# quickwit-oss/tantivy

Hardware: AMD Instinct MI355X
Metric: queries_per_sec_2term_AND_bm25_top10 (higher is better)
Workload: dtype u32+f32; 1 GPU; and2: 10000 queries/batch, k=10, one 10M-doc Zipf segment per GPU (256 terms, df_r=0.5N/r, WithFreqs); term ranks ~ Zipf(1); distinct_queries=3877, mode=block-max pruned (block_wand_intersection semantics), exchange=single rank: no exchange, segments_per_gpu=1, index_bytes=40381332

## Files before the change

tantivy_amd/csrc/tq_api.cpp:

```cpp
#include "tq_internal.hpp"
#include "../host/bm25.hpp"

namespace tqi {

thread_local std::string g_last_error;

int fail(int code, const char *fmt, ...) {
  char buf[512];
  va_list ap;
  va_start(ap, fmt);
  vsnprintf(buf, sizeof buf, fmt, ap);
  va_end(ap);
  g_last_error = buf;
  return code;
}
}

int tq_internal_fail(int code, const char *where, const char *what) {
  return fail(code, "%s: %s", where, what);
}
bool tq_internal_ctx_has_device(const tq_ctx *ctx, int device) {
  return std::find(ctx->devices.begin(), ctx->devices.end(), device) != ctx->devices.end();
}

extern "C" {

const char *tq_last_error(void) { return g_last_error.c_str(); }

int tq_init(const int *device_ids, int n_devices, tq_ctx **out) {
  if (!out) return fail(TQ_ERR_INVALID, "tq_init: out is null");
  int count = 0;
  hipError_t e = hipGetDeviceCount(&count);
  if (e != hipSuccess || count == 0)
    return fail(TQ_ERR_NO_DEVICE, "tq_init: no HIP device visible (%s)",
                e == hipSuccess ? "count=0" : hipGetErrorString(e));
  tq_ctx *ctx = new tq_ctx();
  if (!device_ids || n_devices <= 0) {
    ctx->devices.push_back(0);
  } else {
    for (int i = 0; i < n_devices; ++i) {
      if (device_ids[i] < 0 || device_ids[i] >= count) {
        delete ctx;
        return fail(TQ_ERR_INVALID, "tq_init: device %d out of range (%d visible)", device_ids[i],
                    count);
      }
      ctx->devices.push_back(device_ids[i]);
    }
  }
  *out = ctx;
  return TQ_OK;
}

void tq_shutdown(tq_ctx *ctx) { delete ctx; }

static int segment_upload_common(tq_ctx *ctx, int device, uint32_t max_doc, const uint8_t *idx,
                                 size_t idx_len, const uint8_t *pos, size_t pos_len,
                                 const uint8_t *fieldnorm, size_t fn_len, uint8_t record_option,
                                 bool from_device, tq_segment **out) {
  if (!ctx || !out || !idx) return fail(TQ_ERR_INVALID, "tq_segment_upload: null argument");
  if (idx_len < 8) return fail(TQ_ERR_FORMAT, "idx sub-file shorter than its 8-byte header");
  if (record_option > TQ_WITH_FREQS_AND_POSITIONS)
    return fail(TQ_ERR_INVALID, "bad record_option %u", record_option);
  if (fieldnorm && fn_len < max_doc)
    return fail(TQ_ERR_FORMAT, "fieldnorm file has %zu bytes for max_doc %u", fn_len, max_doc);
  if (std::find(ctx->devices.begin(), ctx->devices.end(), device) == ctx->devices.end())
    return fail(TQ_ERR_INVALID, "device %d not part of this context", device);
  HIP_TRY(hipSetDevice(device));
  tq_segment *s = new tq_segment();
  s->submit = tq_new_submit_queue();
  if (!s->submit) {
    delete s;
    return fail(TQ_ERR_INVALID, "tq_segment_upload: out of memory");
  }
  s->ctx = ctx;
  s->device = device;
  s->dscratch = ctx->scratch_for(device);
  s->max_doc = max_doc;
  s->record_option = record_option;
  s->idx_len = idx_len;
  s->pos_len = (pos && pos_len) ? pos_len : 0;
  if (!from_device) {
    s->h_idx.assign(idx, idx + idx_len);
    if (pos && pos_len) s->h_pos.assign(pos, pos + pos_len);
  }
  const hipMemcpyKind kind = from_device ? hipMemcpyDeviceToDevice : hipMemcpyHostToDevice;
  auto up = [&](uint8_t **dst, const uint8_t *src, size_t n) -> int {
    HIP_TRY(hipMalloc((void **)dst, n + PAD));
    HIP_TRY(hipMemset(*dst + n, 0, PAD));
    HIP_TRY(hipMemcpy(*dst, src, n, kind));
    return TQ_OK;
  };
  int rc = up(&s->d_idx, idx, idx_len);
  if (rc == TQ_OK && pos && pos_len) rc = up(&s->d_pos, pos, pos_len);
  if (rc == TQ_OK && fieldnorm) rc = up(&s->d_fn, fieldnorm, max_doc);
  if (rc == TQ_OK) {
    hipError_t e = hipStreamCreateWithFlags(&s->stream, hipStreamNonBlocking);
    if (e == hipSuccess) e = hipEventCreateWithFlags(&s->ev_stage_done, hipEventDisableTiming);
    if (e == hipSuccess) e = hipEventCreateWithFlags(&s->ev_fork, hipEventDisableTiming);
    if (e == hipSuccess) e = hipEventCreateWithFlags(&s->ev_join, hipEventDisableTiming);
    if (e == hipSuccess) e = hipEventCreateWithFlags(&s->ev_batch_done, hipEventDisableTiming);
    if (e == hipSuccess) e = hipStreamCreateWithFlags(&s->side_stream, hipStreamNonBlocking);
    if (e == hipSuccess) e = hipStreamCreateWithFlags(&s->copy_stream, hipStreamNonBlocking);
    for (int i = 0; i < 2 && e == hipSuccess; ++i) {
      e = hipEventCreateWithFlags(&s->ev_copy_done[i], hipEventDisableTiming);
      if (e == hipSuccess) e = hipEventCreateWithFlags(&s->ev_buf_free[i], hipEventDisableTiming);
    }
    for (int i = 0; i < tq_segment::kTimingRing; ++i) {
      if (e == hipSuccess) e = hipEventCreate(&s->ev_t0[i]);
      if (e == hipSuccess) e = hipEventCreate(&s->ev_t1[i]);
      if (e == hipSuccess) e = hipEventCreate(&s->ev_k0[i]);
      if (e == hipSuccess) e = hipEventCreate(&s->ev_k1[i]);
    }
    if (e == hipSuccess) e = hipMalloc((void **)&s->d_match_counter, 6u * sizeof(unsigned long long));
    if (e == hipSuccess) e = hipMalloc((void **)&s->d_tp_info, 2 * sizeof(TqpInfo));
    if (e != hipSuccess) rc = fail(TQ_ERR_HIP, "segment setup: %s", hipGetErrorString(e));
  }
  if (rc != TQ_OK) {
    tq_segment_free(s);
    return rc;
  }
  s->dseg.idx = s->d_idx;
  s->dseg.pos = s->d_pos;
  s->dseg.fieldnorm = s->d_fn;
  s->dseg.max_doc = max_doc;
  s->dseg.const_fieldnorm_id = 1;
  s->dseg.min_fieldnorm_id = 1;
  if (fieldnorm && !from_device) {
    uint8_t mn = 255;
    for (uint32_t d = 0; d < max_doc; ++d) mn = fieldnorm[d] < mn ? fieldnorm[d] : mn;
    s->dseg.min_fieldnorm_id = max_doc ? mn : 0;
  } else if (fieldnorm) {
    uint32_t *slot = (uint32_t *)s->d_tp_info;
    uint32_t mn = 255;
    hipError_t e = hipMemcpy(slot, &mn, 4, hipMemcpyHostToDevice);
    if (e == hipSuccess) e = tqp_launch_min_fieldnorm(s->d_fn, max_doc, slot, s->stream);
    if (e == hipSuccess) e = hipMemcpyAsync(&mn, slot, 4, hipMemcpyDeviceToHost, s->stream);
    if (e == hipSuccess) e = hipStreamSynchronize(s->stream);
    if (e != hipSuccess) {
      tq_segment_free(s);
      return fail(TQ_ERR_HIP, "fieldnorm scan: %s", hipGetErrorString(e));
    }
    s->dseg.min_fieldnorm_id = max_doc ? mn : 0;
  }
  {
    uint64_t total_tokens = 0;
    hipError_t e = hipSuccess;
    if (!from_device)
      memcpy(&total_tokens, idx, 8);
    else
      e = hipMemcpy(&total_tokens, s->d_idx, 8, hipMemcpyDeviceToHost);
    const float avg = max_doc ? (float)total_tokens / (float)max_doc : 0.0f;
    if (e == hipSuccess && total_tokens && std::isfinite(avg) && avg > 0.0f) {
      const tantivy_amd::Bm25Weight w = tantivy_amd::Bm25Weight::from_idf(1.0f, avg);
      e = hipMalloc((void **)&s->d_local_cache, 256 * sizeof(float));
      if (e == hipSuccess) e = hipMemcpy(s->d_local_cache, w.cache, 256 * sizeof(float), hipMemcpyHostToDevice);
    }
    if (e != hipSuccess) {
      tq_segment_free(s);
      return fail(TQ_ERR_HIP, "segment cache: %s", hipGetErrorString(e));
    }
  }
  *out = s;
  return TQ_OK;
}

int tq_segment_upload(tq_ctx *ctx, int device, uint32_t max_doc, const uint8_t *idx,
                      size_t idx_len, const uint8_t *pos, size_t pos_len, const uint8_t *fieldnorm,
                      size_t fn_len, uint8_t record_option, tq_segment **out) {
  return segment_upload_common(ctx, device, max_doc, idx, idx_len, pos, pos_len, fieldnorm, fn_len,
                               record_option, false, out);
}

int tq_segment_upload_device(tq_ctx *ctx, int device, uint32_t max_doc, const uint8_t *d_idx,
                             size_t idx_len, const uint8_t *d_pos, size_t pos_len,
                             const uint8_t *d_fieldnorm, size_t fn_len, uint8_t record_option,
                             tq_segment **out) {
  return segment_upload_common(ctx, device, max_doc, d_idx, idx_len, d_pos, pos_len, d_fieldnorm,
                               fn_len, record_option, true, out);
}

int tq_segment_upload_fields(tq_ctx *ctx, int device, uint32_t max_doc, uint32_t n_fields, const tq_field_files *fields,
                             uint8_t record_option, tq_segment **out) {
  if (!ctx || !out || !fields) return fail(TQ_ERR_INVALID, "tq_segment_upload_fields: null argument");
  if (n_fields == 0 || n_fields > TQ_MAX_FIELDS)
    return fail(TQ_ERR_INVALID, "tq_segment_upload_fields: n_fields %u not in 1..%u", n_fields, TQ_MAX_FIELDS);
  if (n_fields == 1)
    return tq_segment_upload(ctx, device, max_doc, fields[0].idx, fields[0].idx_len, fields[0].pos, fields[0].pos_len,
                             fields[0].fieldnorm, fields[0].fn_len, record_option, out);
  uint64_t idx_base[TQ_MAX_FIELDS], pos_base[TQ_MAX_FIELDS], pos_len[TQ_MAX_FIELDS];
  size_t idx_total = 0, pos_total = 0;
  for (uint32_t f = 0; f < n_fields; ++f) {
    const tq_field_files &ff = fields[f];
    if (!ff.idx) return fail(TQ_ERR_INVALID, "tq_segment_upload_fields: field %u: null idx", f);
    if (ff.idx_len < 8) return fail(TQ_ERR_FORMAT, "field %u: idx sub-file shorter than its 8-byte header", f);
    if (ff.fieldnorm && ff.fn_len < max_doc)
      return fail(TQ_ERR_FORMAT, "field %u: fieldnorm file has %zu bytes for max_doc %u", f, ff.fn_len, max_doc);
    pos_len[f] = ff.pos && ff.pos_len ? ff.pos_len : 0;
    idx_base[f] = idx_total;
    pos_base[f] = pos_total;
    idx_total += f + 1 < n_fields ? (ff.idx_len + PAD + 15) & ~(size_t)15 : ff.idx_len;
    pos_total += f + 1 < n_fields && pos_len[f] ? (pos_len[f] + PAD + 15) & ~(size_t)15 : pos_len[f];
  }
  std::vector<uint8_t> idx(idx_total, 0), pos(pos_total, 0);
  for (uint32_t f = 0; f < n_fields; ++f) {
    memcpy(idx.data() + idx_base[f], fields[f].idx, fields[f].idx_len);
    if (pos_len[f]) memcpy(pos.data() + pos_base[f], fields[f].pos, pos_len[f]);
  }
  tq_segment *s = nullptr;
  int rc = segment_upload_common(ctx, device, max_doc, idx.data(), idx_total, pos_total ? pos.data() : nullptr, pos_total,
                                 fields[0].fieldnorm, fields[0].fn_len, record_option, false, &s);
  if (rc != TQ_OK) return rc;
  s->n_fields = n_fields;
  for (uint32_t f = 0; f < n_fields; ++f) {
    s->field_idx_base[f] = idx_base[f];
    s->field_idx_len[f] = fields[f].idx_len;
    s->field_pos_base[f] = pos_base[f];
    s->field_pos_len[f] = pos_len[f];
    if (f == 0 || !fields[f].fieldnorm) continue;
    hipError_t e = hipMalloc((void **)&s->d_fn_field[f], (size_t)max_doc + PAD);
    if (e == hipSuccess) e = hipMemset(s->d_fn_field[f] + max_doc, 0, PAD);
    if (e == hipSuccess) e = hipMemcpy(s->d_fn_field[f], fields[f].fieldnorm, max_doc, hipMemcpyHostToDevice);
    if (e != hipSuccess) {
      tq_segment_free(s);
      return fail(TQ_ERR_HIP, "field %u fieldnorms: %s", f, hipGetErrorString(e));
    }
  }
  *out = s;
  return TQ_OK;
}

void tq_segment_free(tq_segment *s) {
  if (!s) return;
  (void)hipSetDevice(s->device);
  if (s->stream) (void)hipStreamSynchronize(s->stream);
  if (s->batch_in_flight && s->ev_batch_done) (void)hipEventSynchronize(s->ev_batch_done);
  for (void *slab : s->term_slabs) (void)hipFree(slab);
  dense_arena_free(s);
  for (void *ptr : s->dense_extra) (void)hipFree(ptr);
  if (s->d_terms) (void)hipFree(s->d_terms);
  if (s->d_idx) (void)hipFree(s->d_idx);
  if (s->d_pos) (void)hipFree(s->d_pos);
  if (s->d_fn) (void)hipFree(s->d_fn);
  for (uint8_t *fn : s->d_fn_field)
    if (fn) (void)hipFree(fn);
  if (s->d_alive) (void)hipFree(s->d_alive);
  if (s->d_docmat) (void)hipFree(s->d_docmat);
  if (s->d_doccls) (void)hipFree(s->d_doccls);
  if (s->d_tp_info) (void)hipFree(s->d_tp_info);
  if (s->d_local_cache) (void)hipFree(s->d_local_cache);
  if (s->d_match_counter) (void)hipFree(s->d_match_counter);
  s->d_stage.release();
  s->d_misc.release();
  for (int i = 0; i < 2; ++i) {
    s->h_prep_stage[i].release();
    if (s->ev_prep[i]) (void)hipEventDestroy(s->ev_prep[i]);
  }
  if (s->ev_prep_order) (void)hipEventDestroy(s->ev_prep_order);
  s->d_thr.release();
  tq_free_plan_scratch(s->plan);
  s->plan = nullptr;
  tq_free_submit_queue(s->submit);
  s->submit = nullptr;
  s->d_qmatches.release();
  s->d_share_words.release();
  s->d_ashare_words.release();
  s->d_bshare_words.release();
  s->d_count_queries.release();
  s->d_count_out.release();
  s->d_count_bits.release();
  s->d_count_wgs.release();
  s->d_set_work.release();
  free_columns(s);
  s->d_docset_queries.release();
  s->d_docset_counts.release();
  s->d_docset_offs.release();
  s->d_docset_partials.release();
  s->d_docset_starts.release();
  s->d_docset_docs.release();
  s->d_docset_squeries.release();
  s->d_docset_caches.release();
  s->d_docset_scores.release();
  s->d_docset_trees.release();
  s->d_sort_ks.release();
  s->d_sort_partials.release();
  s->d_sort_slice_counts.release();
  s->d_sort_rows.release();
  s->h_sort_ks.release();
  s->d_agg_rows.release();
  s->d_agg_term_rows.release();
  s->d_agg_range_starts.release();
  s->h_agg_range_starts.release();
  s->h_docset.release();
  s->h_stage.release();
  s->h_out.release();
  if (s->side_stream) (void)hipStreamSynchronize(s->side_stream);
  if (s->copy_stream) (void)hipStreamSynchronize(s->copy_stream);
  for (hipEvent_t ev : {s->ev_stage_done, s->ev_fork, s->ev_join, s->ev_batch_done, s->ev_copy_done[0],
                        s->ev_copy_done[1], s->ev_buf_free[0], s->ev_buf_free[1]})
    if (ev) (void)hipEventDestroy(ev);
  if (s->side_stream) (void)hipStreamDestroy(s->side_stream);
  if (s->copy_stream) (void)hipStreamDestroy(s->copy_stream);
  s->d_stage_alt.release();
  for (int i = 0; i < tq_segment::kTimingRing; ++i)
    for (hipEvent_t ev : {s->ev_t0[i], s->ev_t1[i], s->ev_k0[i], s->ev_k1[i]})
      if (ev) (void)hipEventDestroy(ev);
  if (s->stream) (void)hipStreamDestroy(s->stream);
  delete s;
}

}

namespace tqi {
int order_after_last_batch(tq_segment *s, hipStream_t st) {
  if (s->batch_in_flight && s->last_stream != st)
    HIP_TRY(hipStreamWaitEvent(st, s->ev_batch_done, 0));
  return TQ_OK;
}
int wait_segment_idle(tq_segment *s) {
  HIP_TRY(hipStreamSynchronize(s->stream));
  if (s->batch_in_flight) {
    HIP_TRY(hipEventSynchronize(s->ev_batch_done));
    s->batch_in_flight = false;
  }
  return TQ_OK;
}
}

extern "C" {

int tq_segment_set_alive_bitset(tq_segment *s, const uint8_t *bytes, size_t len) {
  if (!s) return fail(TQ_ERR_INVALID, "tq_segment_set_alive_bitset: null segment");
  TQ_SEGMENT_LOCK(s);
  HIP_TRY(hipSetDevice(s->device));
  {
    const int wrc = wait_segment_idle(s);
    if (wrc != TQ_OK) return wrc;
  }
  if (s->d_alive) (void)hipFree(s->d_alive);
  s->d_alive = nullptr;
  s->bytes_alive = 0;
  s->dseg.alive = nullptr;
  if (!bytes) return TQ_OK;
  if (len < 4) return fail(TQ_ERR_FORMAT, "alive bitset shorter than its header");
  const uint32_t max_value = rd32(bytes);
  const size_t need = ((size_t)s->max_doc + 63) / 64 * 8;
  if (max_value != s->max_doc || len - 4 < need || (len - 4) % 8 != 0)
    return fail(TQ_ERR_FORMAT, "alive bitset for %u docs / %zu bytes does not fit max_doc %u",
                max_value, len - 4, s->max_doc);
  HIP_TRY(hipMalloc((void **)&s->d_alive, len - 4 + PAD));
  HIP_TRY(hipMemset(s->d_alive + (len - 4), 0, PAD));
  HIP_TRY(hipMemcpy(s->d_alive, bytes + 4, len - 4, hipMemcpyHostToDevice));
  s->bytes_alive = len - 4;
  s->dseg.alive = s->d_alive;
  s->alive_docs = 0;
  for (uint32_t d = 0; d + 8u <= s->max_doc; d += 8u) s->alive_docs += (uint32_t)__builtin_popcount(bytes[4 + (d >> 3)]);
  if (s->max_doc & 7u) s->alive_docs += (uint32_t)__builtin_popcount(bytes[4 + (s->max_doc >> 3)] & ((1u << (s->max_doc & 7u)) - 1u));
  return TQ_OK;
}

int tq_last_batch_match_counts(tq_segment *s, uint32_t *out, uint32_t n) {
  if (!s || !out) return fail(TQ_ERR_INVALID, "tq_last_batch_match_counts: null argument");
  TQ_SEGMENT_LOCK(s);
  if (n > s->last_batch_queries) return fail(TQ_ERR_INVALID, "the last batch had %u queries", s->last_batch_queries);
  HIP_TRY(hipSetDevice(s->device));
  {
    const int wrc = wait_segment_idle(s);
    if (wrc != TQ_OK) return wrc;
  }
  HIP_TRY(hipMemcpy(out, s->d_qmatches.p, (size_t)n * sizeof(uint32_t), hipMemcpyDeviceToHost));
  return TQ_OK;
}

int tq_last_batch_query_kernels(tq_segment *s, uint32_t *out, uint32_t n) {
  if (!s || !out) return fail(TQ_ERR_INVALID, "tq_last_batch_query_kernels: null argument");
  TQ_SEGMENT_LOCK(s);
  if (!s->opt.record_query_kernels || s->last_query_kernel.size() < n)
    return fail(TQ_ERR_INVALID, "the last batch recorded %zu queries (option \"record_query_kernels\")", s->last_query_kernel.size());
  memcpy(out, s->last_query_kernel.data(), (size_t)n * sizeof(uint32_t));
  return TQ_OK;
}

int tq_count_batch(tq_segment *s, const tq_query *queries, uint32_t n_queries,
                   uint32_t *out_counts) {
  if (!s || (!queries && n_queries) || !out_counts)
    return fail(TQ_ERR_INVALID, "tq_count_batch: null argument");
  TQ_SEGMENT_LOCK(s);
  if (n_queries == 0) return TQ_OK;
  return count_batch(s, queries, n_queries, out_counts);
}

static DocsetCall rows_call(const char *fn, uint32_t *out_docs, float *out_scores, uint64_t out_cap, uint64_t *out_starts) {
  DocsetCall call(fn);
  call.out_docs = out_docs;
  call.out_scores = out_scores;
  call.out_cap = out_cap;
  call.out_starts = out_starts;
  return call;
}

int tq_docset_batch(tq_segment *s, const tq_query *queries, uint32_t n_queries, uint32_t *out_docs, uint64_t out_cap,
                    uint64_t *out_starts) {
  if (!s || (!queries && n_queries) || (!out_docs && out_cap) || !out_starts)
    return fail(TQ_ERR_INVALID, "tq_docset_batch: null argument");
  TQ_SEGMENT_LOCK(s);
  return docset_batch(s, queries, n_queries, rows_call("tq_docset_batch", out_docs, nullptr, out_cap, out_starts));
}

int tq_docset_batch_device(tq_segment *s, const tq_query *queries, uint32_t n_queries, uint32_t *d_out_docs,
                           uint64_t out_cap, uint64_t *d_out_starts, void *hip_stream) {
  if (!s || (!queries && n_queries) || (!d_out_docs && out_cap) || !d_out_starts)
    return fail(TQ_ERR_INVALID, "tq_docset_batch_device: null argument");
  TQ_SEGMENT_LOCK(s);
  DocsetCall call = rows_call("tq_docset_batch_device", d_out_docs, nullptr, out_cap, d_out_starts);
  call.device_out = true;
  call.hip_stream = hip_stream;
  return docset_batch(s, queries, n_queries, call);
}

int tq_docset_scored_batch(tq_segment *s, const tq_query *queries, uint32_t n_queries, uint32_t *out_docs, float *out_scores,
                           uint64_t out_cap, uint64_t *out_starts) {
  if (!s || (!queries && n_queries) || ((!out_docs || !out_scores) && out_cap) || !out_starts)
    return fail(TQ_ERR_INVALID, "tq_docset_scored_batch: null argument");
  TQ_SEGMENT_LOCK(s);
  DocsetCall call = rows_call("tq_docset_scored_batch", out_docs, out_scores, out_cap, out_starts);
  call.scored = true;
  return docset_batch(s, queries, n_queries, call);
}

int tq_docset_scored_batch_device(tq_segment *s, const tq_query *queries, uint32_t n_queries, uint32_t *d_out_docs,
                                  float *d_out_scores, uint64_t out_cap, uint64_t *d_out_starts, void *hip_stream) {
  if (!s || (!queries && n_queries) || ((!d_out_docs || !d_out_scores) && out_cap) || !d_out_starts)
    return fail(TQ_ERR_INVALID, "tq_docset_scored_batch_device: null argument");
  TQ_SEGMENT_LOCK(s);
  DocsetCall call = rows_call("tq_docset_scored_batch_device", d_out_docs, d_out_scores, out_cap, d_out_starts);
  call.scored = call.device_out = true;
  call.hip_stream = hip_stream;
  return docset_batch(s, queries, n_queries, call);
}

int tq_last_batch_stats(tq_segment *s, tq_batch_stats *out) {
  if (!s || !out) return fail(TQ_ERR_INVALID, "tq_last_batch_stats: null argument");
  TQ_SEGMENT_LOCK(s);
  HIP_TRY(hipSetDevice(s->device));
  if (s->stats_pending) {
    {
      const int wrc = wait_segment_idle(s);
      if (wrc != TQ_OK) return wrc;
    }
    unsigned long long m = 0;
    if (s->stats_sorted) {
      unsigned long long t[3] = {0, 0, 0};
      HIP_TRY(hipMemcpy(t, s->d_match_counter, sizeof t, hipMemcpyDeviceToHost));
      m = t[0];
      s->stats.matches = m;
      s->stats.algorithmic_bytes += 8u * t[1] + (s->stats_sorted_optional ? 8u * t[0] : 0u) + 13u * t[2];
      if (s->stats_agg_metric) {
        unsigned long long b[2] = {0, 0};
        HIP_TRY(hipMemcpy(b, s->d_match_counter + 3, sizeof b, hipMemcpyDeviceToHost));
        s->stats.algorithmic_bytes += 8u * b[0] + (s->stats_agg_metric_optional ? 8u * b[1] : 0u);
      }
      if (s->stats_agg_terms) {
        unsigned long long e = 0;
        HIP_TRY(hipMemcpy(&e, s->d_match_counter + 3, sizeof e, hipMemcpyDeviceToHost));
        s->stats.algorithmic_bytes += 12u * e;
        if (s->stats_agg_terms_sub) {
          unsigned long long b[2] = {0, 0};
          HIP_TRY(hipMemcpy(b, s->d_match_counter + 4, sizeof b, hipMemcpyDeviceToHost));
          s->stats.algorithmic_bytes += 40u * e + 8u * b[0] + (s->stats_agg_metric_optional ? 8u * b[1] : 0u);
        }
        if (s->stats_agg_terms_hist_row) {
          unsigned long long b[2] = {0, 0};
          HIP_TRY(hipMemcpy(b, s->d_match_counter + 4, sizeof b, hipMemcpyDeviceToHost));
          s->stats.algorithmic_bytes += 4u * (uint64_t)(s->stats_agg_terms_hist_row - 1u) * e + 8u * b[0] + (s->stats_agg_metric_optional ? 8u * b[1] : 0u);
        }
      }
      s->stats_sorted = false;
    } else {
      HIP_TRY(hipMemcpy(&m, s->d_match_counter, sizeof m, hipMemcpyDeviceToHost));
      s->stats.matches = m;
      s->stats.algorithmic_bytes += m * s->stats_match_bytes;
    }
    if (s->opt.timing) {
      uint64_t first = s->batches_reported;
      if (s->batches_timed - first > (uint64_t)tq_segment::kTimingRing)
        first = s->batches_timed - tq_segment::kTimingRing;
      double k_sum = 0, t_sum = 0;
      uint32_t n = 0;
      for (uint64_t b = first; b < s->batches_timed; ++b) {
        const int i = (int)(b % tq_segment::kTimingRing);
        float km = 0, tm = 0;
        if (hipEventElapsedTime(&km, s->ev_k0[i], s->ev_k1[i]) == hipSuccess &&
            hipEventElapsedTime(&tm, s->ev_t0[i], s->ev_t1[i]) == hipSuccess) {
          k_sum += km;
          t_sum += tm;
          ++n;
        }
      }
      s->batches_reported = s->batches_timed;
      if (n) {
        s->stats.kernel_ms = (float)(k_sum / n);
        s->stats.total_ms = (float)(t_sum / n);
      }
      s->stats.batches_averaged = n;
    }
    s->stats.host_plan_ms = s->host_ms_n ? (float)(s->host_ms_sum / s->host_ms_n) : 0.0f;
    s->host_ms_sum = 0;
    s->host_ms_n = 0;
    s->stats_pending = false;
  }
  *out = s->stats;
  return TQ_OK;
}

int tq_segment_reserve_columns(tq_segment *s, const uint64_t *postings_offs, uint32_t n) {
  if (!s || (!postings_offs && n)) return fail(TQ_ERR_INVALID, "tq_segment_reserve_columns: null argument");
  TQ_SEGMENT_LOCK(s);
  if (!s->terms.empty())
    return fail(TQ_ERR_INVALID, "tq_segment_reserve_columns: call it before the first tq_term_prepare");
  s->reserved_cols.clear();
  for (uint32_t i = 0; i < n && i < TQD_MAT_SLOTS; ++i) s->reserved_cols[postings_offs[i]] = true;
  s->cols_reserved = true;
  return TQ_OK;
}

int tq_segment_get_stats(tq_segment *s, tq_segment_stats *out) {
  if (!s || !out) return fail(TQ_ERR_INVALID, "tq_segment_get_stats: null argument");
  TQ_SEGMENT_LOCK(s);
  tq_segment_stats r{};
  r.index_bytes = s->idx_len;
  r.positions_bytes = s->pos_len;
  r.fieldnorm_bytes = s->d_fn ? s->max_doc : 0;
  r.alive_bytes = s->bytes_alive;
  r.term_table_bytes = s->bytes_term_tables + s->d_terms_cap * sizeof(TqdTerm);
  r.bitmap_bytes = s->bytes_bitmaps;
  r.docmat_bytes = s->bytes_docmat;
  r.posdir_bytes = s->bytes_posdir;
  r.scratch_bytes = s->d_stage.cap + s->d_stage_alt.cap + s->d_misc.cap + s->d_thr.cap + s->d_qmatches.cap + s->d_share_words.cap +
                    s->d_ashare_words.cap + s->d_bshare_words.cap + s->d_count_queries.cap + s->d_count_out.cap +
                    s->d_count_bits.cap + s->d_count_wgs.cap + s->d_set_work.cap + s->docset_scratch_bytes();
  {
    std::lock_guard<std::mutex> lk(s->dscratch->m);
    r.device_scratch_bytes = s->dscratch->partials.cap + s->dscratch->share_stage.cap + s->dscratch->ashare_stage.cap +
                             s->dscratch->bshare_stage.cap;
  }
  r.n_terms = (uint32_t)s->terms.size();
  r.n_dense_lists = s->n_dense_lists;
  r.n_docmat_columns = s->n_mat_slots;
  r.probe_evictions = (uint32_t)std::min<uint64_t>(s->probe_evictions, 0xFFFFFFFFull);
  r.dense_budget_bytes = s->dense_budget();
  r.lead_mat_bytes = s->lmat_bytes_total;
  r.lead_mat_stale = s->lmat_stale_skips;
  *out = r;
  return TQ_OK;
}

int tq_set_option(tq_segment *s, const char *name, int64_t value) {
  if (!s || !name) return fail(TQ_ERR_INVALID, "tq_set_option: null argument");
  TQ_SEGMENT_LOCK(s);
  if (!strcmp(name, "exhaustive"))
    __atomic_store_n(&s->opt.exhaustive, value != 0 ? 1 : 0, __ATOMIC_RELAXED);
  else if (!strcmp(name, "timing"))
    s->opt.timing = value != 0;
  else if (!strcmp(name, "use_dpp"))
    s->opt.use_dpp = value != 0;
  else if (!strcmp(name, "use_dense"))
    s->opt.use_dense = value != 0;
  else if (!strcmp(name, "or_windows"))
    s->opt.or_windows = value < 0 ? -1 : (value != 0);
  else if (!strcmp(name, "dense_ratio") && value >= 1)
    s->opt.dense_ratio = (int)value;
  else if (!strcmp(name, "rdir_budget_x") && value >= 0 && value <= 0x7FFFFFFF)
    s->opt.rdir_budget_x = (int)value;
  else if (!strcmp(name, "lead_mat_budget_x") && value >= 0 && value <= 0x7FFFFFFF)
    s->opt.lead_mat_budget_x = (int)value;
  else if (!strcmp(name, "lead_mat_cut") && value >= 1 && value <= 0x7FFFFFFF)
    s->opt.lead_mat_cut = (int)value;
  else if (!strcmp(name, "probe_budget_x") && value >= 0 && value <= 0x7FFFFFFF)
    s->opt.probe_budget_x = (int)value, s->probe_full = false;
  else if (!strcmp(name, "dense_budget_x") && value >= 0)
    s->opt.dense_budget_x = (int)value;
  else if (!strcmp(name, "bound_slack_ppm") && value >= 0 && value <= 1000000000)
    __atomic_store_n(&s->opt.bound_slack_ppm, (int)value, __ATOMIC_RELAXED);
  else if (!strcmp(name, "dense"))
    s->opt.dense = value != 0;
  else if (!strcmp(name, "docmat"))
    s->opt.docmat = value != 0;
  else if (!strcmp(name, "docsig"))
    s->opt.docsig = value != 0;
  else if (!strcmp(name, "device_prepare"))
    s->opt.device_prepare = value != 0;
  else if (!strcmp(name, "xunion_ratio") && value >= 0 && value <= 0x7FFFFFFF)
    s->opt.xunion_ratio = (int)value;
  else if (!strcmp(name, "count_bitmap_ratio") && value >= 0 && value <= 0x7FFFFFFF)
    s->opt.count_bitmap_ratio = (int)value;
  else if (!strcmp(name, "docset_temp_lists") && value >= 0 && value <= 0x7FFFFFFF)
    s->opt.docset_temp_lists = (int)value;
  else if (!strcmp(name, "docset_trees") && (value == 0 || value == 1))
    s->opt.docset_trees = (int)value;
  else if (!strcmp(name, "docset_score_trees") && (value == 0 || value == 1))
    s->opt.docset_score_trees = (int)value;
  else if (!strcmp(name, "sort_slices") && value >= 0 && value <= 256)
    s->opt.sort_slices = (int)value;
  else if (!strcmp(name, "agg_slices") && value >= 0 && value <= 256)
    s->opt.agg_slices = (int)value;
  else if (!strcmp(name, "agg_lds_buckets") && value >= 0 && value <= (int64_t)tqk_agg_lds_buckets())
    s->opt.agg_lds_buckets = (int)value;
  else if (!strcmp(name, "ashare_inline_warm") && value >= 0 && value <= 2)
    s->opt.ashare_inline_warm = (int)value;
  else if (!strcmp(name, "ashare_min_batch") && value >= 0 && value <= 0x7FFFFFFF)
    s->opt.ashare_min_batch = (int)value;
  else if (!strcmp(name, "xunion_min_queries") && value >= 1 && value <= 0x7FFFFFFF)
    s->opt.xunion_min_queries = (int)value;
  else if (!strcmp(name, "record_query_kernels"))
    s->opt.record_query_kernels = value != 0;
  else if (!strcmp(name, "debug") && value >= -1 && value <= 0x7FFFFFFF)
    s->opt.debug = (int)value;
  else if (!strcmp(name, "submit_window_us") && value >= 0 && value <= 1000000)
    s->opt.submit_window_us = (int)value;
  else
    return fail(TQ_ERR_INVALID, "unknown option '%s'", name);
  return TQ_OK;
}

int tq_decode_postings(tq_segment *s, tq_term_handle term, uint32_t *docs, uint32_t *tfs) {
  if (!s || !docs || !tfs) return fail(TQ_ERR_INVALID, "tq_decode_postings: null argument");
  TQ_SEGMENT_LOCK(s);
  if (term >= s->terms.size()) return fail(TQ_ERR_INVALID, "unknown term handle %u", term);
  if (s->terms[term].set_kind != TermHost::kNoSet) return fail(TQ_ERR_INVALID, "tq_decode_postings: handle %u is a term set: it has no postings", term);
  HIP_TRY(hipSetDevice(s->device));
  int rc = sync_terms(s, s->stream);
  if (rc != TQ_OK) return rc;
  const TermHost &t = s->terms[term];
  const size_t bytes = (size_t)t.doc_freq * sizeof(uint32_t);
  rc = s->d_misc.ensure(2 * bytes + 64);
  if (rc != TQ_OK) return rc;
  uint32_t *dd = (uint32_t *)s->d_misc.p, *dt = dd + t.doc_freq;
  hipError_t e = tqk_launch_decode_list(s->dseg, s->d_terms, term, t.n_blocks, dd, dt,
                                        s->opt.use_dpp != 0, s->stream);
  if (e != hipSuccess) return fail(TQ_ERR_HIP, "decode launch: %s", hipGetErrorString(e));
  HIP_TRY(hipMemcpyAsync(docs, dd, bytes, hipMemcpyDeviceToHost, s->stream));
  HIP_TRY(hipMemcpyAsync(tfs, dt, bytes, hipMemcpyDeviceToHost, s->stream));
  HIP_TRY(hipStreamSynchronize(s->stream));
  return TQ_OK;
}

int tq_decode_position_deltas(tq_segment *s, tq_term_handle term, uint32_t *out, uint64_t cap,
                              uint64_t *n_out) {
  if (!s || !n_out) return fail(TQ_ERR_INVALID, "tq_decode_position_deltas: null argument");
  TQ_SEGMENT_LOCK(s);
  if (term >= s->terms.size()) return fail(TQ_ERR_INVALID, "unknown term handle %u", term);
  const TermHost &t = s->terms[term];
  if (t.set_kind != TermHost::kNoSet) return fail(TQ_ERR_INVALID, "tq_decode_position_deltas: handle %u is a term set: it has no positions", term);
  if (t.positions_len == 0) return fail(TQ_ERR_UNSUPPORTED, "term has no positions on the device");
  *n_out = t.n_positions;
  const uint64_t n = std::min<uint64_t>(cap, t.n_positions);
  if (n == 0 || !out) return TQ_OK;
  HIP_TRY(hipSetDevice(s->device));
  int rc = sync_terms(s, s->stream);
  if (rc != TQ_OK) return rc;
  rc = s->d_misc.ensure(n * sizeof(uint32_t));
  if (rc != TQ_OK) return rc;
  hipError_t e = tqk_launch_decode_positions(s->dseg, s->d_terms, term, (uint32_t *)s->d_misc.p, n,
                                             s->stream);
  if (e != hipSuccess) return fail(TQ_ERR_HIP, "decode launch: %s", hipGetErrorString(e));
  HIP_TRY(hipMemcpyAsync(out, s->d_misc.p, n * sizeof(uint32_t), hipMemcpyDeviceToHost, s->stream));
  HIP_TRY(hipStreamSynchronize(s->stream));
  return TQ_OK;
}

namespace {
struct TableSpan {
  const void *p = nullptr;
  size_t bytes = 0;
  bool host = false;
};
bool table_span(tq_segment *s, uint32_t term, uint32_t which, TableSpan &sp) {
  if (which >= TQ_TABLE_DOCMAT) {
    const size_t per_doc = (size_t)s->max_doc * sizeof(uint64_t);
    switch (which) {
      case TQ_TABLE_DOCMAT: sp = {s->d_docmat, s->d_docmat ? per_doc : 0, false}; return true;
      case TQ_TABLE_DOCCLS: sp = {s->d_doccls, s->d_doccls ? per_doc : 0, false}; return true;
      case TQ_TABLE_LOCAL_CACHE: sp = {s->d_local_cache, s->d_local_cache ? 256 * sizeof(float) : 0, false}; return true;
      case TQ_TABLE_MIN_FIELDNORM_ID: sp = {&s->dseg.min_fieldnorm_id, sizeof(uint32_t), true}; return true;
      default: return false;
    }
  }
  const TermHost &t = s->terms[term];
  const TqdTerm &d = s->h_dterms[term];
  const size_t n_words = bitmap_words(s);
  const size_t n_dir = ((size_t)t.doc_freq + 3) / 4 + 1;
// ... 185 lines not shown
```

tantivy_amd/csrc/tq_count.cpp:

```cpp
#include "tq_internal.hpp"

#include <deque>
#include <unordered_map>

namespace tqi {

int parse_flat_clauses(tq_segment *s, const tq_query &q, FlatClauses &fc, const char **why) {
  fc.n_cl = fc.n_must = fc.n_should = 0;
  fc.empty = fc.all_based = fc.all_boost_mixed = false;
  fc.msm = 0;
  *why = "";
  if (query_has_all(q)) {
    AllForm f;
    const int arc = all_query_form(q, f, why);
    if (arc != TQ_OK) return arc == TQ_ERR_UNSUPPORTED ? FLAT_UNSUPPORTED : FLAT_INVALID;
    AllView v;
    all_strip_view(q, f, v);
    const int prc = parse_flat_clauses(s, v.q, fc, why);
    if (prc != FLAT_OK) return prc;
    for (uint32_t c = 0; c < fc.n_cl; ++c)
      for (uint32_t i = 0; i < fc.cl[c].n; ++i) fc.cl[c].pos[i] = v.pos[fc.cl[c].pos[i]];
    fc.all_based = f.kind == TQ_ALL_BASED;
    fc.all_base = f.base;
    fc.all_boost_mixed = f.boost_mixed;
    return FLAT_OK;
  }
  fc.msm = q.mode == TQ_MODE_BOOL ? q.min_should_match : 0u;
  if (!q.terms || q.n_terms == 0 || q.n_terms > TQ_MAX_TERMS) return *why = "n_terms out of range (1..TQ_MAX_TERMS) or no terms", FLAT_INVALID;
  if (q.mode == TQ_MODE_PHRASE) return *why = "a phrase query", FLAT_UNSUPPORTED;
  if (q.mode > TQ_MODE_BOOL) return *why = "unknown mode", FLAT_INVALID;
  if (q.mode == TQ_MODE_BOOL && !q.occurs) return *why = "TQ_MODE_BOOL without occurs", FLAT_INVALID;
  if (bool_query_is_tree(q)) return *why = "a nested boolean query", FLAT_UNSUPPORTED;
  FlatClauses::Clause *cl = fc.cl;
  uint32_t n_cl = 0;
  for (uint32_t i = 0; i < q.n_terms; ++i) {
    uint32_t occur = q.mode == TQ_MODE_AND ? TQ_MUST : TQ_SHOULD;
    uint32_t id = i;
    if (q.mode == TQ_MODE_BOOL) {
      occur = q.occurs[i];
      if (occur > TQ_MUST_NOT) return *why = "occur out of range", FLAT_INVALID;
      if (q.clause_of) id = q.clause_of[i];
    }
    uint32_t c = 0;
    while (c < n_cl && cl[c].id != id) ++c;
    if (c == n_cl) {
      cl[n_cl] = FlatClauses::Clause{};
      cl[n_cl].id = id;
      cl[n_cl].occur = occur;
      ++n_cl;
    } else if (cl[c].occur != occur) {
      return *why = "mixed occurs in one clause", FLAT_INVALID;
    }
    const uint32_t h = q.terms[i];
    if (h == TQ_TERM_ABSENT) continue;
    if (h >= s->terms.size()) return *why = "term handle out of range", FLAT_INVALID;
    cl[c].pos[cl[c].n] = i;
    cl[c].terms[cl[c].n++] = h;
    cl[c].cost += s->terms[h].doc_freq;
  }
  fc.n_cl = n_cl;
  for (uint32_t c = 0; c < n_cl; ++c) {
    if (cl[c].occur == TQ_MUST) {
      if (cl[c].n == 0) fc.empty = true;
      ++fc.n_must;
    } else if (cl[c].n) {
      if (cl[c].occur == TQ_SHOULD) ++fc.n_should;
    }
  }
  return FLAT_OK;
}

bool count_expression(tq_segment *s, const tq_query &q, TqkCountQuery &cq, bool &known, uint64_t &driver_postings,
                      std::unordered_map<uint32_t, uint32_t> &temp_slot, uint32_t max_temp) {
  known = false;
  driver_postings = 0;
  cq = TqkCountQuery{};
  FlatClauses fc;
  const char *why;
  if (parse_flat_clauses(s, q, fc, &why) != FLAT_OK) return false;
  using Clause = FlatClauses::Clause;
  const Clause *cl = fc.cl;
  const uint32_t n_cl = fc.n_cl, n_must = fc.n_must, n_should = fc.n_should;
  bool empty = fc.empty;
  for (uint32_t c = 0; c < n_cl; ++c)
    for (uint32_t i = 0; i < cl[c].n; ++i) {
      const uint32_t h = cl[c].terms[i];
      if (!expression_bitmap(s, s->terms[h]) && !temp_slot.count(h) && temp_slot.size() >= max_temp) return false;
    }
  if (fc.all_based) return false;
  uint32_t msm = fc.msm;
  if (msm > n_should) empty = true;
  bool should_is_must = false;
  if (!empty && msm >= 2) {
    if (msm != n_should) return false;
    should_is_must = true;
    msm = 0;
  }
  if (n_must == 0 && n_should == 0) empty = true;
  if (empty) {
    known = true;
    return true;
  }
  uint32_t n = 0;
  uint64_t must_cost = ~0ull, should_cost = 0;
  auto put = [&](const Clause &c, uint32_t kind, bool clause_union) {
    for (uint32_t i = 0; i < c.n; ++i) {
      const TermHost &th = s->terms[c.terms[i]];
      if (expression_bitmap(s, th)) {
        cq.dense[n] = (const uint2 *)th.dense_blob;
      } else {
        const uint32_t slot = temp_slot.emplace(c.terms[i], (uint32_t)temp_slot.size()).first->second;
        cq.dense[n] = (const uint2 *)(uintptr_t)slot;
        cq.narrow |= 1u << n;
      }
      cq.kinds |= kind << (2u * n);
      if (kind == TQK_COUNT_MUST && (!clause_union || i + 1 == c.n)) cq.clause_end |= 1u << n;
      ++n;
    }
  };
  const bool has_must = n_must > 0 || should_is_must;
  for (uint32_t c = 0; c < n_cl; ++c) {
    if (cl[c].occur == TQ_MUST || (should_is_must && cl[c].occur == TQ_SHOULD && cl[c].n)) {
      put(cl[c], TQK_COUNT_MUST, true);
      must_cost = std::min(must_cost, cl[c].cost);
    }
  }
  for (uint32_t c = 0; c < n_cl; ++c)
    if (cl[c].occur == TQ_MUST_NOT && cl[c].n) put(cl[c], TQK_COUNT_NOT, false);
  if (!should_is_must)
    for (uint32_t c = 0; c < n_cl; ++c)
      if (cl[c].occur == TQ_SHOULD && cl[c].n) {
        if (has_must && msm == 0) continue;
        put(cl[c], TQK_COUNT_SHOULD, false);
        should_cost += cl[c].cost;
      }
  cq.n_terms = n;
  cq.flags = (has_must ? TQK_COUNT_HAS_MUST : 0u) | ((has_must && msm == 1) ? TQK_COUNT_NEED_SHOULD : 0u);
  driver_postings = has_must ? must_cost : should_cost;
  return true;
}

int count_batch(tq_segment *s, const tq_query *queries, uint32_t n_queries, uint32_t *out_counts) {
  static const uint32_t kRatioEnv = tune_u32("TQ_COUNT_BITMAP_RATIO", 0xFFFFFFFFu);
  const uint32_t kRatio = kRatioEnv != 0xFFFFFFFFu ? kRatioEnv : (uint32_t)s->opt.count_bitmap_ratio;
  static const uint64_t kTempBudget = (uint64_t)std::max<uint32_t>(1u, tune_u32("TQ_COUNT_TEMP_MB", 1024)) << 20;
  const uint32_t n_words = (uint32_t)(((uint64_t)s->max_doc + 31u) / 32u);
  const uint32_t words_per_list = (n_words + 63u) & ~63u;
  const uint32_t max_temp = (uint32_t)std::min<uint64_t>(4096u, kTempBudget / ((uint64_t)words_per_list * 4u));
  std::vector<TqkCountQuery> cqs;
  std::vector<uint32_t> bitmap_q, scan_q, all_q;
  std::unordered_map<uint32_t, uint32_t> temp_slot, trial;
  std::deque<AllView> views;
  std::vector<tq_query> eff;
  std::vector<uint8_t> done;
  const tq_query *const given = queries;
  s->last_batch_slop = false;
  for (uint32_t qi = 0; qi < n_queries; ++qi) {
    if (!query_has_all(given[qi])) continue;
    if (eff.empty()) {
      eff.assign(given, given + n_queries);
      done.assign(n_queries, 0);
    }
    AllForm f;
    const char *why = "";
    const int arc = all_query_form(given[qi], f, &why);
    if (arc != TQ_OK) return fail(arc, "tq_count_batch: query %u: %s", qi, why);
    views.emplace_back();
    all_strip_view(given[qi], f, views.back());
    eff[qi] = views.back().q;
    if (f.kind != TQ_ALL_BASED) continue;
    done[qi] = 1;
    bool any_not = false;
    for (uint32_t i = 0; i < given[qi].n_terms; ++i) {
      if (!((f.keep_mask >> i) & 1u)) continue;
      if (given[qi].terms[i] >= s->terms.size()) return fail(TQ_ERR_INVALID, "tq_count_batch: query %u: term handle out of range", qi);
      any_not = any_not || (given[qi].occurs && given[qi].occurs[i] == TQ_MUST_NOT);
    }
    if (f.min_should == 0 && !any_not)
      out_counts[qi] = s->d_alive ? s->alive_docs : s->max_doc;
    else
      all_q.push_back(qi);
  }
  if (!eff.empty()) queries = eff.data();
  for (uint32_t qi = 0; qi < n_queries; ++qi) {
    if (!given[qi].slop) continue;
    SlopView sv;
    const int vrc = slop_view(s, given[qi], qi, "tq_count_batch", sv, false);
    if (vrc != TQ_OK) return vrc;
    if (done.empty()) done.assign(n_queries, 0);
    done[qi] = 1;
    all_q.push_back(qi);
  }
  std::vector<uint8_t> set_q;
  for (uint32_t qi = 0; s->n_set_slots && qi < n_queries; ++qi) {
    bool has = false;
    const int src = check_set_query(s, given[qi], qi, "tq_count_batch", &has);
    if (src != TQ_OK) return src;
    if (has && set_q.empty()) set_q.assign(n_queries, 0);
    if (has) set_q[qi] = 1;
  }
  for (uint32_t qi = 0; s->n_field_terms && qi < n_queries; ++qi)
    if (query_names_field(s, given[qi])) {
      const int frc = check_field_query(s, given[qi], qi, "tq_count_batch");
      if (frc != TQ_OK) return frc;
    }
  for (uint32_t qi = 0; qi < n_queries; ++qi) {
    if (!done.empty() && done[qi]) continue;
    TqkCountQuery cq;
    bool known = false;
    uint64_t driver = 0;
    trial = temp_slot;
    const bool names_set = !set_q.empty() && set_q[qi];
    const bool expr = (kRatio || names_set) && count_expression(s, queries[qi], cq, known, driver, trial, max_temp);
    if (expr && known) {
      out_counts[qi] = 0;
    } else if (expr && (names_set || driver * kRatio >= (uint64_t)cq.n_terms * s->max_doc)) {
      cqs.push_back(cq);
      bitmap_q.push_back(qi);
      temp_slot.swap(trial);
    } else if (names_set) {
      TqkDocsetQuery dq;
      const char *why = "";
      const int drc = docset_expression(s, given[qi], dq, &why);
      if (drc != FLAT_OK) return fail(drc == FLAT_UNSUPPORTED ? TQ_ERR_UNSUPPORTED : TQ_ERR_INVALID, "tq_count_batch: query %u: %s", qi, why);
      all_q.push_back(qi);
    } else {
      scan_q.push_back(qi);
    }
  }
  HIP_TRY(hipSetDevice(s->device));
  uint32_t mask = 0;
  uint64_t algo_bytes = 0;
  if (!scan_q.empty()) {
    const uint32_t n = (uint32_t)scan_q.size();
    std::vector<tq_query> qs(n);
    for (uint32_t i = 0; i < n; ++i) {
      qs[i] = queries[scan_q[i]];
      qs[i].k = 1;
    }
    std::vector<float> sc(n);
    std::vector<uint32_t> dc(n), ct(n), mc(n);
    CallOpts co;
    int rc = resolve_opts(s, nullptr, co);
    if (rc != TQ_OK) return rc;
    co.exhaustive = true;
    rc = search_batch_host(s, qs.data(), n, 1, sc.data(), dc.data(), ct.data(), co);
    if (rc != TQ_OK) return rc;
    rc = tq_last_batch_match_counts(s, mc.data(), n);
    if (rc != TQ_OK) return rc;
    for (uint32_t i = 0; i < n; ++i) out_counts[scan_q[i]] = mc[i];
    mask = s->stats.kernel_mask;
    algo_bytes = s->stats.algorithmic_bytes;
  } else {
    const int wrc = wait_segment_idle(s);
    if (wrc != TQ_OK) return wrc;
  }
  if (!bitmap_q.empty()) {
    const uint32_t n = (uint32_t)bitmap_q.size();
    int rc = s->d_count_queries.ensure((size_t)n * sizeof(TqkCountQuery));
    if (rc == TQ_OK) rc = s->d_count_out.ensure((size_t)n * sizeof(uint32_t));
    if (rc != TQ_OK) return rc;
    if (!temp_slot.empty()) {
      const int src = sync_terms(s, s->stream);
      if (src != TQ_OK) return src;
      std::vector<uint4> wgs;
      for (const auto &kv : temp_slot) push_scatter_work(wgs, s, kv.first, kv.second);
      rc = s->d_count_bits.ensure((size_t)temp_slot.size() * words_per_list * sizeof(uint32_t));
      if (rc == TQ_OK) rc = s->d_count_wgs.ensure(wgs.size() * sizeof(uint4));
      if (rc != TQ_OK) return rc;
      HIP_TRY(hipMemsetAsync(s->d_count_bits.p, 0, (size_t)temp_slot.size() * words_per_list * sizeof(uint32_t), s->stream));
      HIP_TRY(hipMemcpyAsync(s->d_count_wgs.p, wgs.data(), wgs.size() * sizeof(uint4), hipMemcpyHostToDevice, s->stream));
      const hipError_t se = tqk_launch_count_scatter(s->dseg, s->d_terms, (const uint4 *)s->d_count_wgs.p, (uint32_t)wgs.size(),
                                                     (uint32_t *)s->d_count_bits.p, words_per_list, s->stream);
      if (se != hipSuccess) return fail(TQ_ERR_HIP, "count scatter launch: %s", hipGetErrorString(se));
      for (TqkCountQuery &cq : cqs)
        for (uint32_t m = 0; m < cq.n_terms; ++m)
          if ((cq.narrow >> m) & 1u)
            cq.dense[m] = (const uint2 *)((const uint32_t *)s->d_count_bits.p + (size_t)(uintptr_t)cq.dense[m] * words_per_list);
    }
    HIP_TRY(hipMemcpyAsync(s->d_count_queries.p, cqs.data(), (size_t)n * sizeof(TqkCountQuery), hipMemcpyHostToDevice, s->stream));
    HIP_TRY(hipMemsetAsync(s->d_count_out.p, 0, (size_t)n * sizeof(uint32_t), s->stream));
    TqkCountParams p{};
    p.queries = (const TqkCountQuery *)s->d_count_queries.p;
    p.alive = s->d_alive;
    p.out_counts = (uint32_t *)s->d_count_out.p;
    p.n_queries = n;
    p.n_words = n_words;
    const hipError_t e = tqk_launch_count_bitmaps(p, s->stream);
    if (e != hipSuccess) return fail(TQ_ERR_HIP, "count kernel launch: %s", hipGetErrorString(e));
    std::vector<uint32_t> got(n);
    HIP_TRY(hipMemcpyAsync(got.data(), s->d_count_out.p, (size_t)n * sizeof(uint32_t), hipMemcpyDeviceToHost, s->stream));
    HIP_TRY(hipStreamSynchronize(s->stream));
    for (uint32_t i = 0; i < n; ++i) {
      out_counts[bitmap_q[i]] = got[i];
      algo_bytes += (uint64_t)cqs[i].n_terms * p.n_words * 4u;
    }
    mask |= TQ_KERNEL_COUNT_BITMAPS;
  }
  if (!all_q.empty()) {
    const uint32_t n = (uint32_t)all_q.size();
    std::vector<tq_query> qs(n);
    for (uint32_t i = 0; i < n; ++i) qs[i] = given[all_q[i]];
    std::vector<uint64_t> starts((size_t)n + 1u);
    DocsetCall call("tq_count_batch", DocsetConsumer::kCount);
    call.out_starts = starts.data();
    call.caller_q = all_q.data();
    call.n_caller = n_queries;
    const int rc = docset_batch(s, qs.data(), n, call);
// ... 15 lines not shown
```

tantivy_amd/csrc/tq_docset.cpp:

```cpp
#include "tq_internal.hpp"

#include <deque>
#include <unordered_map>

namespace tqi {

int docset_expression(tq_segment *s, const tq_query &q, TqkDocsetQuery &dq, const char **why, FlatClauses *fc_out) {
  dq = TqkDocsetQuery{};
  FlatClauses fc_own;
  FlatClauses &fc = fc_out ? *fc_out : fc_own;
  const int prc = parse_flat_clauses(s, q, fc, why);
  if (prc != FLAT_OK) return prc;
  using Clause = FlatClauses::Clause;
  if (fc.empty_set()) {
    dq.min_should = 1;
    return FLAT_OK;
  }
  const bool should_is_must = fc.should_is_must();
  const uint32_t msm = should_is_must ? 0u : fc.msm;
  const bool has_must = fc.n_must > 0 || should_is_must || fc.all_based;
  uint32_t n = 0;
  auto put = [&](const Clause &c, uint32_t kind) {
    for (uint32_t i = 0; i < c.n; ++i) {
      const TermHost &th = s->terms[c.terms[i]];
// ... 374 lines not shown
    if (b.tree_bytes) memcpy(h_tq, b.tqs.data(), b.tree_bytes);
    if (tree_map_bytes) {
      uint32_t *const map = (uint32_t *)(h_tq + b.tree_bytes);
      for (const DocsetSubBatch &sb : b.cut.subs)
        for (uint32_t t = sb.t0; t < sb.t1; ++t) map[t] = b.tree_q[t] - sb.q0;
    }
    if (slop_bytes) memcpy(h_tq + b.slop_off, b.slop_qs.data(), slop_bytes);
    HIP_TRY(hipMemcpyAsync(s->d_docset_trees.p, h_tq, tree_blob_bytes, hipMemcpyHostToDevice, st));
  }
  if (call.consumer == Consumer::kSort) rc = sort_prepare(s, *call.sort, b.queries, n_queries, b.cut.max_sub_n, b.n_words, st);
  if (call.consumer == Consumer::kAgg) rc = agg_prepare(s, *call.agg, n_queries, b.cut.max_sub_n, b.n_words, st);
  if (rc != TQ_OK) return rc;
  if (slop_bytes) {
    HIP_TRY(hipMemsetAsync(s->d_slop_over.p, 0, (size_t)b.n_over_words() * sizeof(uint32_t), st));
    s->last_batch_slop = true;
  }
  return TQ_OK;
}

int launch_match_bits(const Batch &b, const DocsetSubBatch &sb) {
  tq_segment *const s = b.s;
  if (sb.wg1 > sb.wg0) {
    HIP_TRY(hipMemsetAsync(s->d_count_bits.p, 0, (size_t)sb.n_temp * b.words_per_list * sizeof(uint32_t), b.st));
    const int rc = launched(tqk_launch_count_scatter(s->dseg, s->d_terms, (const uint4 *)s->d_count_wgs.p + sb.wg0, (uint32_t)(sb.wg1 - sb.wg0),
                                                     (uint32_t *)s->d_count_bits.p, b.words_per_list, b.st), "doc-set scatter");
    if (rc != TQ_OK) return rc;
  }
  if (sb.t1 > sb.t0) {
    TqkDocsetTreeParams tp{};
    tp.seg = s->dseg;
    tp.terms = s->d_terms;
    tp.queries = (const TqdTreeQuery *)s->d_docset_trees.p + sb.t0;
    tp.table_base = (const uint8_t *)s->share_table_lo;
    tp.bits = (uint32_t *)s->d_count_bits.p;
    tp.n_queries = sb.t1 - sb.t0;
    tp.n_words = b.n_words;
    tp.words_per_list = b.words_per_list;
    tp.any_phrase = sb.any_phrase ? 1u : 0u;
    const int rc = launched(tqk_launch_docset_tree(tp, b.st), "doc-set tree");
    if (rc != TQ_OK) return rc;
  }
  if (sb.s1 > sb.s0) {
    TqkPhraseSlopParams pp{};
    pp.seg = s->dseg;
    pp.terms = s->d_terms;
    pp.queries = (const TqdSlopQuery *)((const uint8_t *)s->d_docset_trees.p + b.slop_off) + sb.s0;
    pp.table_base = (const uint8_t *)s->share_table_lo;
    pp.overflow = (uint32_t *)s->d_slop_over.p;
    pp.bits = (uint32_t *)s->d_count_bits.p;
    pp.n_queries = sb.s1 - sb.s0;
    pp.n_words = b.n_words;
    pp.words_per_list = b.words_per_list;
    for (uint32_t k = sb.s0; k < sb.s1; ++k) (b.slop_qs[k].n_terms > 2u ? pp.any_carry : pp.any_pair) = 1u;
    return launched(tqk_launch_phrase_slop_bits(pp, b.st), "sloppy phrase");
  }
  return TQ_OK;
}

hipError_t launch_scores(const Batch &b, const DocsetSubBatch &sb, const TqkDocsetParams &p, float *d_scores) {
  tq_segment *const s = b.s;
  TqkScoreParams sp{};
  sp.seg = s->dseg;
  sp.terms = s->d_terms;
  sp.caches = (const float *)s->d_docset_caches.p;
  sp.out_docs = p.out_docs;
  sp.out_scores = d_scores;
  sp.out_cap = p.out_cap;
  sp.n_tiles = b.n_tiles;
  sp.any_blocks = sb.score_blocks ? 1u : 0u;
  hipError_t e = hipSuccess;
  uint32_t r0 = sb.q0;
  for (uint32_t t = sb.t0; t <= sb.t1 && e == hipSuccess; ++t) {
    const uint32_t r1 = t < sb.t1 ? b.tree_q[t] : sb.q1;
    if (r1 > r0) {
      sp.queries = (const TqkScoreQuery *)s->d_docset_squeries.p + r0;
      sp.tile_counts = p.tile_counts + (size_t)(r0 - sb.q0) * b.n_tiles;
      sp.tile_offs = p.tile_offs + (size_t)(r0 - sb.q0) * b.n_tiles;
      sp.n_queries = r1 - r0;
      if (b.score_fields) {
        TqkScoreFieldsParams fp{};
        fp.base = sp;
        fp.fn[0] = s->d_fn;
        for (uint32_t f = 1; f < TQK_MAX_FIELDS; ++f) fp.fn[f] = s->d_fn_field[f];
        e = tqk_launch_docset_score_fields(fp, b.st);
      } else {
        e = tqk_launch_docset_score(sp, b.st);
      }
    }
    r0 = r1 + 1u;
  }
  if (e != hipSuccess || sb.t1 == sb.t0) return e;
  TqkDocsetTreeScoreParams tsp{};
  tsp.seg = s->dseg;
  tsp.terms = s->d_terms;
  tsp.queries = (const TqdTreeQuery *)s->d_docset_trees.p + sb.t0;
  tsp.query_of = (const uint32_t *)((const uint8_t *)s->d_docset_trees.p + b.tree_bytes) + sb.t0;
  tsp.caches = sp.caches;
  tsp.table_base = (const uint8_t *)s->share_table_lo;
  tsp.tile_counts = p.tile_counts;
  tsp.tile_offs = p.tile_offs;
  tsp.out_docs = p.out_docs;
  tsp.out_scores = d_scores;
  tsp.out_cap = p.out_cap;
  tsp.n_queries = sb.t1 - sb.t0;
  tsp.n_tiles = b.n_tiles;
  tsp.any_phrase = sb.any_phrase ? 1u : 0u;
  return tqk_launch_docset_tree_score(tsp, b.st);
}

int launch_consumer(const Batch &b, const DocsetSubBatch &sb, uint32_t stages, uint32_t *d_docs, float *d_scores, uint64_t cap) {
  static const uint32_t kStageMin = tune_u32("TQ_DOCSET_STAGE_MIN", 2048);
  tq_segment *const s = b.s;
  TqkDocsetParams p{};
  p.queries = (const TqkDocsetQuery *)s->d_docset_queries.p + sb.q0;
  p.alive = s->d_alive;
  p.tile_counts = (uint32_t *)s->d_docset_counts.p;
  p.tile_offs = (uint64_t *)s->d_docset_offs.p;
  p.partials = (uint64_t *)s->d_docset_partials.p;
  p.base_in = sb.q0 ? b.d_starts + sb.q0 : nullptr;
  p.out_starts = b.d_starts + sb.q0;
  p.query_sizes = (uint32_t *)s->d_qmatches.p + sb.q0;
  p.total_out = s->d_match_counter;
  p.out_docs = d_docs;
  p.out_cap = cap;
  p.n_queries = sb.q1 - sb.q0;
  p.n_tiles = b.n_tiles;
  p.n_words = b.n_words;
  p.max_doc = s->max_doc;
  p.stage_min_docs = kStageMin;
  if (b.call.consumer == Consumer::kSort) return sort_launch(s, *b.call.sort, p, sb.q0, b.st);
  if (b.call.consumer == Consumer::kAgg) return agg_launch(s, *b.call.agg, p, sb.q0, b.st);
  hipError_t e = hipSuccess;
  if (stages & DS_COUNT) {
    e = tqk_launch_docset_count(p, b.st);
    if (e == hipSuccess) e = tqk_launch_docset_scan(p, b.st);
  }
  if (e == hipSuccess && (stages & DS_WRITE)) e = tqk_launch_docset_write(p, b.st);
  if (e == hipSuccess && (stages & DS_WRITE) && b.call.scored) e = launch_scores(b, sb, p, d_scores);
  return launched(e, "doc-set kernel");
}

int sweep(const Batch &b, uint32_t stages, uint32_t *d_docs, float *d_scores, uint64_t cap) {
  for (const DocsetSubBatch &sb : b.cut.subs) {
    int rc = (stages & DS_SCATTER) ? launch_match_bits(b, sb) : TQ_OK;
    if (rc == TQ_OK) rc = launch_consumer(b, sb, stages, d_docs, d_scores, cap);
    if (rc != TQ_OK) return rc;
  }
  return TQ_OK;
}

int run_device(const Batch &b) {
  tq_segment *const s = b.s;
  const DocsetCall &call = b.call;
  if (b.timed) HIP_TRY(hipEventRecord(s->ev_k0[b.ring], b.st));
  int rc = sweep(b, DS_SCATTER | DS_COUNT | DS_WRITE, call.out_docs, call.out_scores, call.out_cap);
  if (rc == TQ_OK && call.consumer == Consumer::kAgg) rc = agg_finish(s, *call.agg, b.n_queries, b.st);
  if (rc != TQ_OK) return rc;
  if (b.timed) {
    HIP_TRY(hipEventRecord(s->ev_k1[b.ring], b.st));
    HIP_TRY(hipEventRecord(s->ev_t1[b.ring], b.st));
    ++s->batches_timed;
  }
  s->stats_pending = true;
  s->stats_match_bytes = call.scored ? 9 : 4;
  s->stats_sorted = !b.own_passes();
  s->stats_sorted_optional = (call.sort && call.sort->optional) || (call.agg && call.agg->optional);
  s->stats_agg_metric = call.agg && call.agg->metric;
  s->stats_agg_metric_optional = call.agg && call.agg->metric_optional;
  s->stats_agg_terms = call.agg && call.agg->terms;
  s->stats_agg_terms_sub = call.agg && call.agg->terms_sub;
  s->stats_agg_terms_hist_row = call.agg && call.agg->terms_hist ? call.agg->plan.n_buckets + 1u : 0u;
  HIP_TRY(hipEventRecord(s->ev_batch_done, b.st));
  s->last_stream = b.st;
  s->batch_in_flight = true;
  return TQ_OK;
}

int run_host(const Batch &b) {
  tq_segment *const s = b.s;
  const DocsetCall &call = b.call;
  const std::vector<DocsetSubBatch> &subs = b.cut.subs;
  int rc = sweep(b, DS_SCATTER | DS_COUNT, nullptr, nullptr, 0);
  if (rc != TQ_OK) return rc;
  HIP_TRY(hipMemcpyAsync(call.out_starts, b.d_starts, ((size_t)b.n_queries + 1u) * sizeof(uint64_t), hipMemcpyDeviceToHost, b.st));
  HIP_TRY(hipStreamSynchronize(b.st));
  const uint64_t total = call.out_starts[b.n_queries];
  s->stats.matches = total;
  if (call.consumer == Consumer::kCount) return slop_overflow_readback(s, call.fn);
  s->stats.algorithmic_bytes += (call.scored ? 9u : 4u) * total;
  if (total > call.out_cap)
    return fail(TQ_ERR_INVALID, "%s: the batch has %llu docs, out_cap is %llu (out_starts is filled: retry with that many)", call.fn,
                (unsigned long long)total, (unsigned long long)call.out_cap);
  if (!total) return slop_overflow_readback(s, call.fn);
  rc = s->d_docset_docs.ensure((size_t)total * sizeof(uint32_t));
  if (rc == TQ_OK && call.scored) rc = s->d_docset_scores.ensure((size_t)total * sizeof(float));
  if (rc != TQ_OK) return rc;
  if (subs.size() > 1 && !b.slop_qs.empty())
    HIP_TRY(hipMemsetAsync(s->d_slop_over.p, 0, (size_t)b.n_over_words() * sizeof(uint32_t), b.st));
  rc = sweep(b, subs.size() == 1 ? DS_WRITE : (DS_SCATTER | DS_COUNT | DS_WRITE), (uint32_t *)s->d_docset_docs.p, (float *)s->d_docset_scores.p, total);
  if (rc != TQ_OK) return rc;
  HIP_TRY(hipMemcpyAsync(call.out_docs, s->d_docset_docs.p, (size_t)total * sizeof(uint32_t), hipMemcpyDeviceToHost, b.st));
  if (call.scored) HIP_TRY(hipMemcpyAsync(call.out_scores, s->d_docset_scores.p, (size_t)total * sizeof(float), hipMemcpyDeviceToHost, b.st));
  HIP_TRY(hipStreamSynchronize(b.st));
  if (s->d_docset_docs.cap > ((size_t)256 << 20)) s->d_docset_docs.release();
  if (s->d_docset_scores.cap > ((size_t)256 << 20)) s->d_docset_scores.release();
  return slop_overflow_readback(s, call.fn);
}

}

int docset_batch(tq_segment *s, const tq_query *queries, uint32_t n_queries, const DocsetCall &call) {
  static const uint64_t kTempBudget = (uint64_t)std::max<uint32_t>(1u, tune_u32("TQ_COUNT_TEMP_MB", 1024)) << 20;
  Batch b{s, queries, n_queries, call};
  b.n_words = (uint32_t)(((uint64_t)s->max_doc + 31u) / 32u);
  b.words_per_list = (b.n_words + 63u) & ~63u;
  b.n_tiles = (b.n_words + tqk_docset_tile_words() - 1u) / tqk_docset_tile_words();
  b.max_temp = s->opt.docset_temp_lists > 0
                   ? (uint32_t)s->opt.docset_temp_lists
                   : (uint32_t)std::min<uint64_t>(4096u, kTempBudget / std::max<uint64_t>(1u, (uint64_t)b.words_per_list * 4u));
  b.max_temp = std::max<uint32_t>(b.max_temp, TQ_MAX_TERMS);
  b.max_sub_queries = std::max<uint32_t>(1u, (1u << 26) / std::max(1u, b.n_tiles));
  b.dqs.resize(n_queries);
  b.sqs.resize(call.scored ? n_queries : 0u);
  s->last_batch_slop = false;
  s->slop_over_words = b.n_over_words();
  int rc = check_and_express(b);
  if (rc == TQ_OK) rc = plan_trees(b);
  if (rc != TQ_OK) return rc;
  cut_docset_subs(s, b.dqs, b.sqs, b.tree_q, b.tqs, b.slop_qi, b.slop_qs, b.max_temp, b.max_sub_queries, b.cut);

  HIP_TRY(hipSetDevice(s->device));
  b.st = call.device_out && call.hip_stream ? (hipStream_t)call.hip_stream : s->stream;
  rc = wait_segment_idle(s);
  if (rc != TQ_OK) return rc;
  const bool scored = call.scored;
  s->stats = tq_batch_stats{};
  s->stats.kernel_mask = (call.consumer == Consumer::kSort ? TQ_KERNEL_SORT : call.consumer == Consumer::kAgg ? (call.agg->terms_hist ? TQ_KERNEL_AGG_TERMS_HIST : call.agg->terms_sub ? TQ_KERNEL_AGG_TERMS_SUB : call.agg->terms ? TQ_KERNEL_AGG_TERMS : call.agg->range ? TQ_KERNEL_AGG_RANGE : call.agg->metric ? TQ_KERNEL_AGG_SUB : TQ_KERNEL_AGG) : TQ_KERNEL_DOCSET) |
                         (scored ? TQ_KERNEL_DOCSET_SCORE : 0u) | (b.tqs.empty() ? 0u : TQ_KERNEL_DOCSET_TREE) |
                         (scored && !b.tqs.empty() ? TQ_KERNEL_DOCSET_TREE_SCORE : 0u) | (b.slop_qs.empty() ? 0u : TQ_KERNEL_PHRASE_SLOP);
  s->stats.algorithmic_bytes = b.algo_bytes;
  s->stats_pending = false;
  s->last_batch_queries = 0;
  if (b.own_passes() && (n_queries == 0 || b.n_tiles == 0)) {
    if (call.device_out) {
      HIP_TRY(hipMemsetAsync(call.out_starts, 0, ((size_t)n_queries + 1u) * sizeof(uint64_t), b.st));
    } else {
      memset(call.out_starts, 0, ((size_t)n_queries + 1u) * sizeof(uint64_t));
    }
    return TQ_OK;
  }
  if (!b.cut.wgs.empty() || scored || !b.tqs.empty() || !b.slop_qs.empty()) {
    rc = sync_terms(s, s->stream);
    if (rc != TQ_OK) return rc;
  }
  rc = size_and_upload(b);
  if (rc != TQ_OK) return rc;
  s->last_batch_queries = n_queries;
  return call.device_out ? run_device(b) : run_host(b);
}

}
```

tantivy_amd/csrc/tq_internal.hpp:

```cpp
#pragma once
#include <hip/hip_runtime.h>

#include <algorithm>
#include <array>
#include <atomic>
#include <chrono>
#include <condition_variable>
#include <deque>
#include <map>
#include <mutex>
#include <new>
#include <cstdlib>
#include <cmath>
#include <cstdarg>
#include <cstdio>
#include <cstring>
#include <string>
#include <unordered_map>
#include <unordered_set>
#include <thread>
#include <vector>

#include "../../include/tantivy_amd.h"
#include "tq_device.h"
// ... 18 lines not shown
constexpr size_t PAD = 1088;

struct DevBuf {
  void *p = nullptr;
  size_t cap = 0;
  int ensure(size_t n) {
    if (n <= cap) return TQ_OK;
    const size_t ncap = std::max(n, cap * 2);
    if (p) (void)hipFree(p);
    p = nullptr;
    cap = 0;
    void *np = nullptr;
    HIP_TRY(hipMalloc(&np, ncap));
    p = np;
    cap = ncap;
    return TQ_OK;
  }
  void release() {
    if (p) (void)hipFree(p);
    p = nullptr;
    cap = 0;
  }
};
struct PinnedBuf {
  void *p = nullptr;
  size_t cap = 0;
  int ensure(size_t n) {
    if (n <= cap) return TQ_OK;
    const size_t ncap = std::max(n, cap * 2);
    if (p) (void)hipHostFree(p);
    p = nullptr;
    cap = 0;
    void *np = nullptr;
    HIP_TRY(hipHostMalloc(&np, ncap, hipHostMallocDefault));
    p = np;
    cap = ncap;
    return TQ_OK;
  }
  void release() {
    if (p) (void)hipHostFree(p);
    p = nullptr;
    cap = 0;
  }
};

struct TermHost {
  void *blob = nullptr;
  const TqdTerm *d_self = nullptr;
  void *dense_blob = nullptr;
  void *posdir_blob = nullptr;
  void *tf8_blob = nullptr;
  void *pos_blob = nullptr;
  void *probe_dense_blob = nullptr, *probe_tf8_blob = nullptr;
  void *probe_posdir_blob = nullptr;
  int32_t probe_slot = -1;
  void *rdir_blob = nullptr;
  void *rdir_ent = nullptr;
  uint32_t rdir_shift = 0;
  uint8_t *probe_own_dir = nullptr;
  void *rmax_blob = nullptr;
  uint32_t rmax_list = 255;
  void *flat_blob = nullptr;
  void *lnorm_blob = nullptr;
  void *lmat_blob = nullptr;
  uint64_t lmat_epoch = 0;
  uint32_t doc_freq = 0, n_blocks = 0, n_full = 0, n_tail = 0;
  uint32_t last_doc = 0;
  bool wants_col = true;
  uint64_t postings_len = 0, positions_len = 0;
  uint64_t n_positions = 0;
  enum : uint8_t { kNoSet = 0, kSet = 1, kSetReleased = 2 };
  uint8_t set_kind = kNoSet;
  uint8_t field = 0;
};

inline uint32_t rd32(const uint8_t *p) {
  return (uint32_t)p[0] | ((uint32_t)p[1] << 8) | ((uint32_t)p[2] << 16) | ((uint32_t)p[3] << 24);
}
inline bool read_vint(const uint8_t *d, size_t len, size_t &at, uint64_t &out) {
  uint64_t r = 0;
  unsigned shift = 0;
  while (at < len) {
    uint8_t b = d[at++];
    r |= (uint64_t)(b & 127u) << shift;
    if (b & 128u) {
      out = r;
      return true;
    }
    shift += 7;
    if (shift > 63) return false;
  }
  return false;
}
inline bool read_vint32_block(const uint8_t *d, size_t len, size_t &at, uint32_t &out) {
  uint32_t r = 0, shift = 0;
  while (at < len) {
    uint8_t b = d[at++];
    r += (uint32_t)(b & 127u) << shift;
    if (b & 128u) {
      out = r;
      return true;
    }
    shift += 7;
  }
  return false;
}

struct Options {
  int exhaustive = 0;
  int timing = 0;
  int use_dpp = 1;
  int dense = 1;
  int dense_ratio = TQD_DENSE_RATIO;
  int dense_budget_x = 8;
  int use_dense = 1;
  int docmat = 1;
  int docsig = 1;
  int device_prepare = 0;
  int or_windows = -1;
  int bound_slack_ppm = 0;
  int xunion_ratio = 64;
  int xunion_min_queries = 64;
  int lead_mat_budget_x = 4;
  int lead_mat_cut = 16;
  int rdir_budget_x = 4;
  int probe_budget_x = 16;
  int count_bitmap_ratio = 128;
  int docset_temp_lists = 0;
  int docset_trees = 0;
  int docset_score_trees = 0;
  int sort_slices = 0;
  int agg_slices = 0;
  int agg_lds_buckets = -1;
  int ashare_inline_warm = 1;
  int ashare_min_batch = 16;
  int submit_window_us = 100;
  int record_query_kernels = 0;
  int debug = -1;
};


inline uint32_t tune_u32(const char *name, uint32_t dflt) {
  const char *v = getenv(name);
  return v && *v ? (uint32_t)strtoul(v, nullptr, 10) : dflt;
}

}
using namespace tqi;

struct DeviceScratch {
  std::mutex m;
  DevBuf partials, share_stage, ashare_stage, bshare_stage;
  hipEvent_t ev_last = nullptr;
  hipStream_t last_stream = nullptr;
  bool in_flight = false;
};
struct tq_ctx {
  std::vector<int> devices;
  std::mutex m;
  std::map<int, DeviceScratch *> scratch;
  DeviceScratch *scratch_for(int device) {
    std::lock_guard<std::mutex> lk(m);
    DeviceScratch *&p = scratch[device];
    if (!p) p = new DeviceScratch();
    return p;
  }
  ~tq_ctx() {
    for (auto &kv : scratch) {
      (void)hipSetDevice(kv.first);
      if (kv.second->ev_last) (void)hipEventDestroy(kv.second->ev_last);
      kv.second->partials.release();
      kv.second->share_stage.release();
      kv.second->ashare_stage.release();
      kv.second->bshare_stage.release();
      delete kv.second;
    }
  }
};

struct tq_segment {
  tq_ctx *ctx = nullptr;
  int device = 0;
  hipStream_t stream = nullptr;
  uint32_t max_doc = 0;
  uint8_t record_option = 0;
  std::vector<uint8_t> h_idx, h_pos;
  size_t idx_len = 0, pos_len = 0;
  TqpInfo *d_tp_info = nullptr;
  uint8_t *d_idx = nullptr, *d_pos = nullptr, *d_fn = nullptr, *d_alive = nullptr;
  uint32_t n_fields = 1;
  uint64_t field_idx_base[TQ_MAX_FIELDS] = {}, field_idx_len[TQ_MAX_FIELDS] = {};
  uint64_t field_pos_base[TQ_MAX_FIELDS] = {}, field_pos_len[TQ_MAX_FIELDS] = {};
  uint8_t *d_fn_field[TQ_MAX_FIELDS] = {};
  uint32_t n_field_terms = 0;
  uint8_t prep_field = 0;
  float *d_local_cache = nullptr;
  uint64_t *d_docmat = nullptr;
  uint64_t *d_doccls = nullptr;
  uint32_t n_mat_slots = 0;
  TqdSegment dseg{};
  std::vector<TermHost> terms;
  std::vector<std::pair<void *, size_t>> rdir_chunks;
  uint8_t *rdir_chunk_cur = nullptr;
  size_t rdir_chunk_left = 0;
  bool rdir_span_ok = false;
  std::vector<void *> term_slabs;
  uint8_t *term_slab_cur = nullptr;
  size_t term_slab_left = 0;
  std::vector<TqdTerm> h_dterms;
  TqdTerm *d_terms = nullptr;
  size_t d_terms_cap = 0;
  bool d_terms_dirty = false;
  size_t d_terms_dirty_from = ~(size_t)0;
  size_t d_terms_synced = 0;
  size_t dense_bytes_total = 0;
  uint8_t *dense_arena = nullptr;
  size_t dense_arena_cap = 0, dense_arena_used = 0;
  std::vector<void *> dense_extra;
  bool dense_arena_vmm = false;
  void *dense_arena_va = nullptr;
  size_t dense_arena_mapped = 0, dense_arena_first = 0;
  std::vector<std::pair<hipMemGenericAllocationHandle_t, size_t>> dense_arena_chunks;
  size_t bytes_term_tables = 0, bytes_bitmaps = 0, bytes_docmat = 0, bytes_posdir = 0, bytes_alive = 0;
  uint32_t n_dense_lists = 0;
  uint32_t n_set_slots = 0;
  std::vector<uint32_t> set_free_slots;
  std::vector<void *> set_free_tables;
  DevBuf d_set_work;
  struct ColumnHost {
    bool live = false;
    tq_column_info_t info{};
    TqkColumn dev{};
    void *d_payload = nullptr;
    void *d_blocks = nullptr;
    void *d_present = nullptr;
    uint64_t payload_len = 0;
  };
  ColumnHost columns[TQ_MAX_COLUMNS];
  uint32_t alive_docs = 0;
  std::unordered_map<uint64_t, uint32_t> term_by_off;
  std::unordered_map<uint64_t, bool> reserved_cols;
  bool cols_reserved = false;
  DevBuf d_stage, d_misc, d_thr, d_qmatches;
  DevBuf d_share_words;
  DevBuf d_count_queries, d_count_out, d_count_bits, d_count_wgs;
  DevBuf d_docset_queries, d_docset_counts, d_docset_offs, d_docset_partials, d_docset_starts, d_docset_docs;
  DevBuf d_docset_squeries, d_docset_caches, d_docset_scores;
  DevBuf d_docset_trees;
  DevBuf d_sort_ks, d_sort_partials, d_sort_slice_counts, d_sort_rows;
  PinnedBuf h_sort_ks;
  DevBuf d_agg_rows;
  DevBuf d_agg_term_rows;
  DevBuf d_agg_range_starts;
  PinnedBuf h_agg_range_starts;
  PinnedBuf h_docset;
  size_t docset_scratch_bytes() const {
    return d_docset_queries.cap + d_docset_counts.cap + d_docset_offs.cap + d_docset_partials.cap + d_docset_starts.cap +
           d_docset_docs.cap + d_docset_squeries.cap + d_docset_caches.cap + d_docset_scores.cap +
           d_docset_trees.cap + d_sort_ks.cap + d_sort_partials.cap + d_sort_slice_counts.cap + d_sort_rows.cap + d_agg_rows.cap + d_agg_term_rows.cap +
           d_agg_range_starts.cap;
  }
  DevBuf d_ashare_words, d_bshare_words;
  DeviceScratch *dscratch = nullptr;
  size_t share_span_terms = 0;
  uint64_t share_table_lo = 0;
  bool share_span_ok = true;
  bool lnorm_off = false;
  uint64_t docmat_epoch = 1, docmat_epoch_planned = 0;
  size_t lmat_bytes_total = 0;
  bool lmat_off = false;
  uint32_t lmat_stale_skips = 0;
  uint32_t last_batch_queries = 0;
  DevBuf d_slop_over;
  bool last_batch_slop = false;
  uint32_t slop_over_words = 0;
  std::vector<uint32_t> slop_over_host;
  std::vector<uint32_t> last_query_kernel;
  PinnedBuf h_stage, h_out;
  static constexpr int kTimingRing = 16;
  hipEvent_t ev_stage_done = nullptr, ev_fork = nullptr, ev_join = nullptr;
  hipEvent_t ev_batch_done = nullptr;
  hipStream_t last_stream = nullptr;
  bool batch_in_flight = false;
  hipStream_t side_stream = nullptr;
  hipStream_t copy_stream = nullptr;
  DevBuf d_stage_alt;
  hipEvent_t ev_copy_done[2] = {nullptr, nullptr}, ev_buf_free[2] = {nullptr, nullptr};
  bool buf_used[2] = {false, false};
  uint64_t batches_enqueued = 0;
  hipEvent_t ev_t0[kTimingRing] = {}, ev_t1[kTimingRing] = {}, ev_k0[kTimingRing] = {},
             ev_k1[kTimingRing] = {};
  uint64_t batches_timed = 0, batches_reported = 0;
  bool stage_in_flight = false;
  double host_ms_sum = 0;
  uint32_t host_ms_n = 0;
  unsigned long long *d_match_counter = nullptr;
  Options opt;
  size_t dense_budget() const { return (size_t)opt.dense_budget_x * (idx_len + pos_len + max_doc); }
  size_t probe_budget() const { return (size_t)opt.probe_budget_x * (idx_len + pos_len + max_doc); }
  size_t rdir_budget() const { return (size_t)opt.rdir_budget_x * (idx_len + pos_len + max_doc); }
  size_t rdir_bytes_total = 0;
  PinnedBuf h_prep_stage[2];
  hipEvent_t ev_prep[2] = {nullptr, nullptr}, ev_prep_order = nullptr;
  bool prep_used[2] = {false, false};
  uint32_t prep_calls = 0;
  int prep_pending = -1;
  std::vector<uint32_t> prep_lmax_handles[2];
  const uint32_t *prep_lmax_host[2] = {nullptr, nullptr};
  size_t probe_bytes_total = 0;
  bool probe_full = false;
  struct ProbeSlot {
    uint8_t *base = nullptr;
    uint32_t owner = 0xFFFFFFFFu;
    uint64_t last_batch = 0;
  };
  std::vector<ProbeSlot> probe_slots;
  size_t probe_slot_bytes = 0, probe_bm_bytes = 0, probe_tf_cap = 0, probe_dir_cap = 0, probe_rm_bytes = 0;
  uint64_t probe_batch = 1;
  uint64_t probe_evictions = 0;
  uint64_t probe_replaced_batch = 0;
  uint32_t probe_replaced_n = 0;
  uint64_t probe_no_room_batch = 0;
  bool probe_waited = false;
  bool device_prepare() const { return h_idx.empty() || opt.device_prepare != 0; }
  tq_batch_stats stats{};
  bool stats_pending = false;
  uint32_t stats_match_bytes = 1;
  bool stats_sorted = false, stats_sorted_optional = false;
  bool stats_agg_metric = false, stats_agg_metric_optional = false;
  bool stats_agg_terms = false;
  bool stats_agg_terms_sub = false;
  uint32_t stats_agg_terms_hist_row = 0;
  struct PlanScratch *plan = nullptr;
  std::recursive_mutex exec_m;
  struct SubmitQueue *submit = nullptr;
};

void tq_free_plan_scratch(PlanScratch *p);
void tq_free_submit_queue(struct SubmitQueue *q);
struct SubmitQueue *tq_new_submit_queue();
#define TQ_SEGMENT_LOCK(seg) std::lock_guard<std::recursive_mutex> tq_exec_lock_((seg)->exec_m)

namespace tqi {

template <typename T>
class PodVec {
 public:
  PodVec() = default;
  PodVec(const PodVec &) = delete;
  PodVec &operator=(const PodVec &) = delete;
  PodVec(PodVec &&o) noexcept : p_(o.p_), n_(o.n_), cap_(o.cap_) { o.p_ = nullptr, o.n_ = o.cap_ = 0; }
  PodVec &operator=(PodVec &&o) noexcept {
    swap(o);
    return *this;
  }
  ~PodVec() { free(p_); }
  size_t size() const { return n_; }
  bool empty() const { return n_ == 0; }
  T *data() { return p_; }
  const T *data() const { return p_; }
  T &operator[](size_t i) { return p_[i]; }
  const T &operator[](size_t i) const { return p_[i]; }
  T &back() { return p_[n_ - 1]; }
  const T &back() const { return p_[n_ - 1]; }
  T *begin() { return p_; }
  T *end() { return p_ + n_; }
  const T *begin() const { return p_; }
  const T *end() const { return p_ + n_; }
  void clear() { n_ = 0; }
  void reserve(size_t n) {
    if (n <= cap_) return;
    const size_t ncap = std::max(n, cap_ * 2);
    T *np = (T *)malloc(ncap * sizeof(T));
    if (!np) throw std::bad_alloc();
    if (n_) memcpy(np, p_, n_ * sizeof(T));
    free(p_);
    p_ = np;
    cap_ = ncap;
  }
  void resize(size_t n) {
    reserve(n);
    n_ = n;
  }
  void push_back(const T &v) {
    if (n_ == cap_) reserve(n_ + 1);
    p_[n_++] = v;
  }
  void append(const T *first, const T *last) {
    const size_t n = (size_t)(last - first);
    reserve(n_ + n);
    if (n) memcpy(p_ + n_, first, n * sizeof(T));
    n_ += n;
  }
  void swap(PodVec &o) {
    std::swap(p_, o.p_);
    std::swap(n_, o.n_);
    std::swap(cap_, o.cap_);
  }

 private:
  T *p_ = nullptr;
  size_t n_ = 0, cap_ = 0;
};

struct Group {
  int mode;
  PodVec<TqdQuery> queries;
  std::vector<uint32_t> out_index;
  std::vector<uint32_t> tile_starts;
  std::vector<uint4> chunk_recs;
  std::vector<uint32_t> tile_cost;
  std::vector<TqdTreeQuery> tree;
  std::vector<TqdAllQuery> all;
  std::vector<TqdSlopQuery> slop;
  uint32_t total_tiles = 0, n_chunks = 0, max_k = 1;
  uint64_t list_entries = 0;
  int kpl = 1;
  size_t o_queries = 0, o_tiles = 0, o_outidx = 0, o_chunks = 0, o_sinks = 0;
  size_t o_xqueries = 0;
  size_t o_leads = 0, o_tasks = 0, o_lists = 0;
  void reset() {
    queries.clear();
    out_index.clear();
    tile_starts.clear();
    chunk_recs.clear();
    tile_cost.clear();
    tree.clear();
    all.clear();
    slop.clear();
    total_tiles = 0;
    n_chunks = 0;
    list_entries = 0;
    max_k = 1;
    kpl = 1;
    o_queries = o_tiles = o_outidx = o_chunks = o_sinks = o_xqueries = 0;
    o_leads = o_tasks = o_lists = 0;
  }
};

}

struct alignas(128) PlanSlab {
  size_t q0 = 0, q1 = 0;
  std::vector<uint32_t> starts, slice, query;
// ... 546 lines not shown
```

tantivy_amd/csrc/tq_phrase_slop.cpp:

```cpp
#include "tq_internal.hpp"

namespace tqi {

static_assert(TQK_SLOP_CARRY_CAP == TQ_SLOP_CARRY_CAP, "the kernels' cap is the header's");
static_assert(TQ_SLOP_CARRY_CAP >= 32u, "the contract promises at least 32 entries");
static_assert(TQK_SLOP_MAX_TERMS == 8u, "device phrases take 2..8 terms");

int slop_view(const tq_segment *s, const tq_query &q, uint32_t qi, const char *fn, SlopView &out, bool scored) {
  if (q.mode != TQ_MODE_PHRASE)
    return fail(TQ_ERR_INVALID, "%s: query %u: slop %u outside TQ_MODE_PHRASE (only a PhraseQuery has a slop)", fn, qi, q.slop);
  if (q.slop > TQ_MAX_SLOP)
    return fail(TQ_ERR_UNSUPPORTED, "%s: query %u: slop %u above TQ_MAX_SLOP (%u)", fn, qi, q.slop, TQ_MAX_SLOP);
  if (q.n_terms < 2 || q.n_terms > TQ_MAX_TERMS || !q.terms || !q.phrase_offsets)
    return fail(TQ_ERR_INVALID, "%s: query %u: a phrase needs >= 2 terms and offsets", fn, qi);
  if (q.n_terms > TQK_SLOP_MAX_TERMS)
    return fail(TQ_ERR_UNSUPPORTED, "%s: query %u: device phrases take at most %u terms", fn, qi, TQK_SLOP_MAX_TERMS);
  if (scored && (!q.weights || !std::isfinite(q.weights[0])))
    return fail(TQ_ERR_INVALID, "%s: query %u: a phrase needs a finite weight in weights[0]", fn, qi);
  for (uint32_t i = 0; i < q.n_terms; ++i) {
    const uint32_t h = q.terms[i];
    if (h == TQ_TERM_ABSENT) continue;
    if (h == TQ_TERM_ALL) return fail(TQ_ERR_INVALID, "%s: query %u: a match-all clause inside a phrase", fn, qi);
    if (h >= s->terms.size()) return fail(TQ_ERR_INVALID, "%s: query %u: unknown term handle %u", fn, qi, h);
    if (is_term_set(s, h)) return fail(TQ_ERR_INVALID, "%s: query %u: a term set inside a phrase", fn, qi);
    if (term_field_of(s, h))
      return fail(TQ_ERR_UNSUPPORTED, "%s: query %u: a sloppy phrase over terms of field %u stays on the CPU (field 0 only)", fn, qi, term_field_of(s, h));
  }
  uint32_t order[TQ_MAX_TERMS];
  for (uint32_t i = 0; i < q.n_terms; ++i) order[i] = i;
  auto df = [&](uint32_t i) { return q.terms[i] == TQ_TERM_ABSENT ? 0u : s->terms[q.terms[i]].doc_freq; };
  std::stable_sort(order, order + q.n_terms, [&](uint32_t x, uint32_t y) { return df(x) < df(y); });
  tq_query ordered = q;
  for (uint32_t i = 0; i < q.n_terms; ++i) {
    out.terms[i] = q.terms[order[i]];
    out.offsets[i] = q.phrase_offsets[order[i]];
  }
  ordered.terms = out.terms;
  ordered.phrase_offsets = out.offsets;
  ordered.slop = 0;
  docset_tree_view(ordered, out.v, scored);
  return TQ_OK;
}

int plan_slop_query(tq_segment *s, const tq_query &view, uint32_t qi, uint32_t slop, TqdSlopQuery &sq, uint64_t &qbytes, bool result_bitmap) {
  TqdTreeQuery tq;
  uint64_t list_bytes = 0;
  const int rc = plan_tree_query(s, view, qi, tq, list_bytes, s->share_table_lo);
  if (rc != TQ_OK) return rc;
  sq = TqdSlopQuery{};
  sq.k = view.k;
  sq.slop = slop;
  sq.out_q = qi;
  if (tq.n_terms == 0) return TQ_OK;
  if (tq.n_clauses != 1 || tq.n_terms < 2 || tq.n_terms > TQK_SLOP_MAX_TERMS)
    return fail(TQ_ERR_INVALID, "query %u: a sloppy phrase came out of the tree planner as %u clauses of %u terms", qi, tq.n_clauses, tq.n_terms);
  sq.n_terms = tq.n_terms;
  sq.weight_bits = tq.weight_bits[0];
  for (uint32_t t = 0; t < tq.n_terms; ++t) {
    sq.dense_off[t] = tq.dense_off[t];
    sq.tf8_off[t] = tq.tf8_off[t];
    sq.dir_off[t] = tq.dir_off[t];
    sq.phrase_off[t] = tq.phrase_off[t];
    sq.handle[t] = tq.handle[t];
  }
  const uint64_t n_words = (s->max_doc + 31u) / 32u;
  qbytes += (uint64_t)(tq.n_terms + (result_bitmap ? 2u : 1u)) * n_words * 4u;
  return TQ_OK;
}

int slop_overflow_fail(const char *fn, uint32_t qi, uint32_t docs) {
  return fail(TQ_ERR_UNSUPPORTED, "%s: query %u: carried position list over TQ_SLOP_CARRY_CAP (%u entries) in %u candidate doc%s: its rows are not valid, the query stays on the CPU",
              fn, qi, TQ_SLOP_CARRY_CAP, docs, docs == 1u ? "" : "s");
}

int slop_overflow_verdict(const char *fn, const uint32_t *over, uint32_t n_queries) {
  for (uint32_t qi = 0; qi < n_queries; ++qi)
    if (over[qi]) return slop_overflow_fail(fn, qi, over[qi]);
  return TQ_OK;
}

int slop_overflow_readback(tq_segment *s, const char *fn) {
  if (!s->last_batch_slop) return TQ_OK;
  std::vector<uint32_t> over(s->slop_over_words);
  HIP_TRY(hipMemcpy(over.data(), s->d_slop_over.p, over.size() * sizeof(uint32_t), hipMemcpyDeviceToHost));
  return slop_overflow_verdict(fn, over.data(), (uint32_t)over.size());
}

}

extern "C" int tq_last_batch_slop_overflows(tq_segment *s, uint32_t *out, uint32_t n) {
  using namespace tqi;
  if (!s || !out) return fail(TQ_ERR_INVALID, "tq_last_batch_slop_overflows: null argument");
  TQ_SEGMENT_LOCK(s);
  const uint32_t had = s->slop_over_words;
  if (n > had) return fail(TQ_ERR_INVALID, "the last batch had %u queries", had);
  if (!s->last_batch_slop) {
    memset(out, 0, (size_t)n * sizeof(uint32_t));
    return TQ_OK;
  }
  HIP_TRY(hipSetDevice(s->device));
  {
    const int wrc = wait_segment_idle(s);
    if (wrc != TQ_OK) return wrc;
  }
  HIP_TRY(hipMemcpy(out, s->d_slop_over.p, (size_t)n * sizeof(uint32_t), hipMemcpyDeviceToHost));
  return TQ_OK;
}
```

tantivy_amd/csrc/tq_search.cpp:

```cpp
#include "tq_internal.hpp"

namespace tqi {
namespace {

using Clock = std::chrono::steady_clock;

struct Knobs {
  bool use_bshare = tune_u32("TQ_BSHARE", 1) != 0, bs_rdir = tune_u32("TQ_BS_RDIR", 1) != 0;
  bool use_ashare = tune_u32("TQ_ASHARE", 1) != 0;
  uint32_t ashare_min = std::max<uint32_t>(1u, tune_u32("TQ_AS_MIN_LEADS", 1));
  bool use_ushare = tune_u32("TQ_USHARE", 1) != 0;
  uint32_t debug = tune_u32("TQ_DEBUG", 0);
};
const Knobs &knobs() {
  static const Knobs k;
  return k;
}

struct Batch {
  tq_segment *s;
  const tq_query *queries;
  uint32_t n_queries, out_stride;
  float *out_scores;
  uint32_t *out_docs, *out_counts;
  void *hip_stream;
  CallOpts co;
  uint32_t *out_segment_ords;
  uint32_t segment_ord;
  bool replan = false;
  hipStream_t st = nullptr;
  bool exhaustive = false, or_windows = false;
  Clock::time_point t0, t_route, t_routed, t_laid, t_waited, t_filled;
  size_t terms_from = 0, terms_to = 0;
  std::vector<const float *> caches;
  uint32_t n_union_queries = 0, n_bool_queries = 0, n_sparse2 = 0;
  uint32_t n_all_queries = 0;
  const uint8_t *set_q = nullptr;
  const uint32_t *slop_q = nullptr;
  bool and_probe = false, ashare_on = false, ashare_and = false;
  uint32_t and_tile_cap = TQD_AND_TILE, dense_min_queries = 1;
  uint64_t unique_bytes = 0, dense_ratio = 0;
  PlanScratch *ps = nullptr;
  Group *groups = nullptr;
  RouteTotals t;
  int cus = 256;
  size_t part_off_bytes[kNGroups] = {}, partial_bytes = 0;
  struct Copy { size_t off; const void *src; size_t bytes; };
  std::vector<Copy> copies;
  size_t stage = 0, o_caches = 0, o_terms = 0;
  int bx = 0;
  const uint8_t *ds = nullptr;
  DeviceScratch *sc = nullptr;
  int slot = 0;
  uint32_t grid[kNGroups] = {};
  std::vector<uint32_t> lmat_fill;
};

}

void update_table_span(tq_segment *s) {
  if (s->share_span_terms == s->terms.size()) return;
  uint64_t lo = ~0ull, hi = 0;
  for (const TermHost &th : s->terms)
    for (const void *ptr : {th.dense_blob, th.tf8_blob, th.probe_dense_blob, th.probe_tf8_blob, th.rmax_blob, th.posdir_blob, th.probe_posdir_blob, th.lnorm_blob, th.lmat_blob})
      if (ptr) {
        lo = std::min<uint64_t>(lo, (uint64_t)ptr);
        hi = std::max<uint64_t>(hi, (uint64_t)ptr);
      }
  if (lo == ~0ull) lo = hi = 8;
  {
    uint64_t lo2 = lo, hi2 = hi;
    for (const auto &ch : s->rdir_chunks) {
      lo2 = std::min<uint64_t>(lo2, (uint64_t)ch.first);
      hi2 = std::max<uint64_t>(hi2, (uint64_t)ch.first + ch.second);
    }
    s->rdir_span_ok = !s->rdir_chunks.empty() && hi2 - (lo2 - 8) < (8ull << 32);
    if (s->rdir_span_ok) {
      lo = lo2;
      hi = hi2;
    }
  }
  s->share_table_lo = (lo - 8) & ~255ull;
  s->share_span_ok = hi - s->share_table_lo < (8ull << 32);
  s->share_span_terms = s->terms.size();
}

namespace {

int sync_term_records(Batch &b) {
  HIP_TRY(hipSetDevice(b.s->device));
  b.st = b.hip_stream ? (hipStream_t)b.hip_stream : b.s->stream;
  prep_apply_lmax(b.s, false);
  if (b.s->prep_pending >= 0) {
    if (b.st != b.s->stream) HIP_TRY(hipStreamWaitEvent(b.st, b.s->ev_prep[b.s->prep_pending], 0));
    b.s->prep_pending = -1;
  }
  if (b.s->d_terms_dirty) {
    const size_t n_terms_now = b.s->h_dterms.size();
    if (b.s->d_terms && n_terms_now <= b.s->d_terms_cap && b.s->d_terms_dirty_from >= b.s->d_terms_synced) {
      b.terms_from = std::min(b.s->d_terms_dirty_from, n_terms_now);
      b.terms_to = n_terms_now;
    } else {
      const int rc = sync_terms(b.s, b.st);
      if (rc != TQ_OK) return rc;
    }
  }
  update_table_span(b.s);
  return TQ_OK;
}

void look_at_queries(Batch &b) {
  if (!b.s->plan) b.s->plan = new PlanScratch();
  b.ps = b.s->plan;
  b.ps->q_cache.resize(b.n_queries);
  const size_t n_terms_known = b.s->terms.size();
  const float *last_tc = nullptr;
  uint32_t last_idx = 0;
  for (uint32_t qi = 0; qi < b.n_queries; ++qi) {
    const tq_query &q = b.queries[qi];
    const float *tc = q.tf_cache;
    uint32_t cache_idx = 0;
    if (tc == last_tc && tc) {
      cache_idx = last_idx;
    } else if (tc) {
      const uint32_t rows = b.s->n_fields;
      for (; cache_idx < b.caches.size(); cache_idx += rows)
        if (b.caches[cache_idx] == tc) break;
      if (cache_idx == b.caches.size())
        for (uint32_t f = 0; f < rows; ++f) b.caches.push_back(tc + (size_t)f * 256u);
      last_tc = tc;
      last_idx = cache_idx;
    }
    b.ps->q_cache[qi] = cache_idx;
    b.n_union_queries += (q.mode == TQ_MODE_OR || (q.mode == TQ_MODE_AND && q.n_terms == 1)) ? 1u : 0u;
    b.n_bool_queries += q.mode == TQ_MODE_BOOL ? 1u : 0u;
    if (q.mode == TQ_MODE_AND && q.n_terms == 2 && q.terms && q.terms[0] < n_terms_known && q.terms[1] < n_terms_known) {
      const TermHost &ta = b.s->terms[q.terms[0]], &tb = b.s->terms[q.terms[1]];
      const TermHost &probed = tb.doc_freq < ta.doc_freq ? ta : tb;
      if (!(probed.dense_blob && probed.tf8_blob) && !(probed.rdir_blob && b.s->rdir_span_ok)) ++b.n_sparse2;
    }
  }
}

int build_flat_probe_tables(Batch &b) {
  static const uint32_t kProbeAnd = tune_u32("TQ_AS_PROBE", 1);
  const bool tables = b.s->opt.use_dense && b.s->opt.dense && b.s->opt.probe_budget_x > 0;
  if (kProbeAnd && !b.exhaustive && tables && b.n_queries >= (uint32_t)b.s->opt.ashare_min_batch)
    b.and_probe = kProbeAnd >= 2 || (uint64_t)b.n_sparse2 * 10u >= b.n_queries;
  probe_begin_batch(b.s);
  if (b.exhaustive || !((knobs().use_bshare && b.n_bool_queries) || b.and_probe) || !tables) return TQ_OK;
  bool built = false;
  for (uint32_t qi = 0; qi < b.n_queries; ++qi) {
    const tq_query &q = b.queries[qi];
    const bool and2 = b.and_probe && q.mode == TQ_MODE_AND && q.n_terms == 2;
    if (!((q.mode == TQ_MODE_BOOL && knobs().use_bshare) || and2) || !q.terms || q.n_terms > TQD_AS_MAX_TERMS || q.k > 128u) continue;
    uint32_t skip = 0xFFFFFFFFu;
    if (and2 && q.terms[0] < b.s->terms.size() && q.terms[1] < b.s->terms.size())
      skip = b.s->terms[q.terms[1]].doc_freq < b.s->terms[q.terms[0]].doc_freq ? 1u : 0u;
    for (uint32_t i = 0; i < q.n_terms; ++i) {
      if (i == skip) continue;
      const uint32_t h = q.terms[i];
      if (h >= b.s->terms.size()) continue;
      const TermHost &th = b.s->terms[h];
      if (th.dense_blob && th.tf8_blob) continue;
      if (and2 && th.rdir_blob && b.s->rdir_span_ok) continue;
      if (and2 && b.s->opt.rdir_budget_x > 0 && th.doc_freq < 256u) continue;
      const bool had = th.probe_dense_blob && th.probe_tf8_blob;
      bool ok = false;
      const int prc = build_probe_tables(b.s, h, &ok);
      if (prc != TQ_OK) return prc;
      built = built || (ok && !had);
    }
  }
  if (built) b.s->share_span_terms = ~(size_t)0;
  return TQ_OK;
}

}

int build_tree_query_probe_tables(tq_segment *s, const tq_query &q, bool *built, bool flat_too) {
  if (!s->opt.use_dense || !s->opt.dense || s->opt.probe_budget_x <= 0) return TQ_OK;
  if (q.mode != TQ_MODE_BOOL || !q.terms || q.n_terms > TQ_MAX_TERMS || !(flat_too || bool_query_is_tree(q))) return TQ_OK;
  for (uint32_t i = 0; i < q.n_terms; ++i) {
    const uint32_t h = q.terms[i];
    if (h >= s->terms.size()) continue;
    const TermHost &th = s->terms[h];
    if (!(th.dense_blob && th.tf8_blob)) {
      const bool had = th.probe_dense_blob && th.probe_tf8_blob;
      bool ok = false;
      const int prc = build_probe_tables(s, h, &ok, true);
      if (prc != TQ_OK) return prc;
      *built = *built || (ok && !had);
    }
    if (q.nested_occurs && q.nested_occurs[i] != 255u && (q.nested_occurs[i] & TQ_NESTED_PHRASE) &&
        !s->terms[h].posdir_blob && !s->terms[h].probe_posdir_blob) {
      bool ok = false;
      const int prc = build_probe_posdir(s, h, &ok);
      if (prc != TQ_OK) return prc;
      *built = *built || ok;
    }
  }
  return TQ_OK;
}
// ... 468 lines not shown
    r.n_tiles = acc_tiles;
  }
  return TQ_OK;
}

int plan_query(const Batch &b, uint32_t qi, Group *groups, RouteTotals &t) {
  int rc = check_query(b, qi);
  if (rc != TQ_OK) return rc;
  const tq_query &q = b.queries[qi];
  Route r;
  r.dq.thr_index = 0xFFFFFFFFu;
  r.dq.k = q.k;
  r.dq.cache_idx = b.ps->q_cache[qi];
  r.qbytes = 8ull * q.k;
  const bool any_absent = std::find(q.terms, q.terms + q.n_terms, TQ_TERM_ABSENT) != q.terms + q.n_terms;
  if (b.slop_q && b.slop_q[qi]) {
    rc = route_slop(b, qi, r, groups[kGSlop]);
  } else if (b.n_all_queries && query_has_all(q)) {
    rc = route_all(b, qi, r, groups[kGAll]);
  } else if (b.set_q && b.set_q[qi]) {
    rc = route_tree(b, qi, r, groups[kGTree]);
  } else if (q.mode == TQ_MODE_BOOL) {
    rc = bool_query_is_tree(q) ? route_tree(b, qi, r, groups[kGTree]) : route_bool(b, qi, r, t);
  } else if (q.mode == TQ_MODE_OR || (q.mode == TQ_MODE_AND && q.n_terms == 1 && !any_absent)) {
    rc = route_union(b, qi, r, groups, t);
  } else if (any_absent) {
    r.group = q.mode == TQ_MODE_AND ? kGAndDense : kGPhrase;
  } else {
    rc = sort_by_doc_freq(b, qi, r);
    if (rc == TQ_OK && q.mode == TQ_MODE_AND) route_and(b, qi, r, t);
    if (rc == TQ_OK && q.mode == TQ_MODE_PHRASE) route_phrase(b, qi, r, t);
  }
  if (rc != TQ_OK) return rc;
  t.algo_bytes += r.qbytes;
  r.dq.n_tiles = r.n_tiles;
  r.dq.mode = (uint32_t)kGroupTraits[r.group].mode;
  Group &g = groups[r.group];
  g.queries.push_back(r.dq);
  g.tile_cost.push_back(r.tile_cost);
  g.out_index.push_back(qi);
  g.max_k = std::max(g.max_k, q.k);
  return TQ_OK;
}

int route_in_slabs(Batch &b, uint32_t q_slabs) {
  std::vector<QuerySlab> &qs = b.ps->q_slabs;
  if (qs.size() < q_slabs) qs.resize(q_slabs);
  parallel_slabs(q_slabs, [&](uint32_t sb) {
    QuerySlab &Q = qs[sb];
    for (int gi = 0; gi < kNGroups; ++gi) {
      Q.groups[gi].reset();
      Q.groups[gi].mode = kGroupTraits[gi].mode;
    }
    Q.t = RouteTotals{};
    Q.rc = TQ_OK;
    const uint32_t q0 = (uint32_t)((uint64_t)b.n_queries * sb / q_slabs), q1 = (uint32_t)((uint64_t)b.n_queries * (sb + 1) / q_slabs);
    for (uint32_t qi = q0; qi < q1; ++qi) {
      Q.rc = plan_query(b, qi, Q.groups, Q.t);
      if (Q.rc != TQ_OK) {
        Q.err = g_last_error;
        break;
      }
    }
  });
  uint32_t thr_base[9] = {0};
  size_t g_base[kNGroups][9] = {};
  for (uint32_t sb = 0; sb < q_slabs; ++sb) {
    if (qs[sb].rc != TQ_OK) {
      g_last_error = qs[sb].err;
      return qs[sb].rc;
    }
    thr_base[sb + 1] = thr_base[sb] + qs[sb].t.n_thr_rows;
    b.t.algo_bytes += qs[sb].t.algo_bytes;
    b.t.n_ashare_ext += qs[sb].t.n_ashare_ext;
    b.t.phrase_all_dense = b.t.phrase_all_dense && qs[sb].t.phrase_all_dense;
    for (int gi = 0; gi < kNGroups; ++gi) g_base[gi][sb + 1] = g_base[gi][sb] + qs[sb].groups[gi].queries.size();
  }
  b.t.n_thr_rows = thr_base[q_slabs];
  for (int gi = 0; gi < kNGroups; ++gi) {
    Group &g = b.groups[gi];
    const size_t total = g_base[gi][q_slabs];
    g.queries.resize(total);
    g.tile_cost.resize(total);
    g.out_index.resize(total);
    for (uint32_t sb = 0; sb < q_slabs; ++sb) g.max_k = std::max(g.max_k, qs[sb].groups[gi].max_k);
    for (uint32_t sb = 0; sb < q_slabs; ++sb) g.tree.insert(g.tree.end(), qs[sb].groups[gi].tree.begin(), qs[sb].groups[gi].tree.end());
    for (uint32_t sb = 0; sb < q_slabs; ++sb) g.all.insert(g.all.end(), qs[sb].groups[gi].all.begin(), qs[sb].groups[gi].all.end());
    for (uint32_t sb = 0; sb < q_slabs; ++sb) g.slop.insert(g.slop.end(), qs[sb].groups[gi].slop.begin(), qs[sb].groups[gi].slop.end());
  }
  parallel_slabs(q_slabs, [&](uint32_t sb) {
    for (int gi = 0; gi < kNGroups; ++gi) {
      const Group &src = qs[sb].groups[gi];
      Group &g = b.groups[gi];
      const size_t at = g_base[gi][sb], n = src.queries.size();
      for (size_t i = 0; i < n; ++i) {
        g.queries[at + i] = src.queries[i];
        if (g.queries[at + i].thr_index != 0xFFFFFFFFu) g.queries[at + i].thr_index += thr_base[sb];
      }
      if (n) {
        memcpy(g.tile_cost.data() + at, src.tile_cost.data(), n * sizeof(uint32_t));
        memcpy(g.out_index.data() + at, src.out_index.data(), n * sizeof(uint32_t));
      }
    }
  });
  return TQ_OK;
}

int route_queries(Batch &b) {
  PlanScratch &ps = *b.ps;
  static const uint32_t kDenseRatioEnv = tune_u32("TQ_XU_RATIO", 0xFFFFFFFFu);
  static const uint32_t kDenseMinEnv = tune_u32("TQ_XU_MIN_QUERIES", 0xFFFFFFFFu);
  b.dense_ratio = kDenseRatioEnv != 0xFFFFFFFFu ? kDenseRatioEnv : (uint32_t)b.s->opt.xunion_ratio;
  b.dense_min_queries = std::max<uint32_t>(1u, kDenseMinEnv != 0xFFFFFFFFu ? kDenseMinEnv : (uint32_t)b.s->opt.xunion_min_queries);
  b.groups = ps.groups;
  for (int gi = 0; gi < kNGroups; ++gi) {
    b.groups[gi].reset();
    b.groups[gi].mode = kGroupTraits[gi].mode;
  }
  ps.xrow_term.clear();
  ps.xrow_of.clear();
  ps.xcache = 0xFFFFFFFFu;
  b.t_route = Clock::now();
  static const uint32_t kQuerySlabMin = tune_u32("TQ_PLAN_QUERY_PAR_MIN", 4096);
  const uint32_t q_slabs = (!b.exhaustive && b.n_queries >= kQuerySlabMin) ? std::min<uint32_t>(plan_threads(), 8u) : 1u;
  if (q_slabs > 1) {
    const int rc = route_in_slabs(b, q_slabs);
    if (rc != TQ_OK) return rc;
  } else {
    for (uint32_t qi = 0; qi < b.n_queries; ++qi) {
      const int rc = plan_query(b, qi, b.groups, b.t);
      if (rc != TQ_OK) return rc;
    }
  }
  b.t_routed = Clock::now();
  Group &d = b.groups[kGXUnion], &o = b.groups[kGUnion];
  if (!d.queries.empty() && d.queries.size() < b.dense_min_queries) {
    o.queries.append(d.queries.begin(), d.queries.end());
    o.tile_cost.insert(o.tile_cost.end(), d.tile_cost.begin(), d.tile_cost.end());
    o.out_index.insert(o.out_index.end(), d.out_index.begin(), d.out_index.end());
    o.max_k = std::max(o.max_k, d.max_k);
    d.reset();
    d.mode = kGroupTraits[kGXUnion].mode;
  }
  return TQ_OK;
}

uint32_t ashare_resident(int cus) {
  static const uint32_t kAGridMul = tune_u32("TQ_AS_GRID_MUL", 0);
  return (uint32_t)std::max(1, cus) * (kAGridMul ? kAGridMul : tqk_ashare_waves_per_cu());
}

int plan_group_tasks(Batch &b) {
  PlanScratch &ps = *b.ps;
  (void)hipDeviceGetAttribute(&b.cus, hipDeviceAttributeMultiprocessorCount, b.s->device);
  const bool alone = std::count_if(b.groups, b.groups + kNGroups, [](const Group &g) { return !g.queries.empty(); }) == 1;
  for (int gi = 0; gi < kNGroups; ++gi) {
    Group &g = b.groups[gi];
    if (g.queries.empty()) continue;
    if (gi == kGTree || gi == kGSlop) {
      const uint32_t tiles = tqk_tree_tiles((b.s->max_doc + 31u) / 32u);
      g.kpl = kpl_for(g.max_k);
      for (TqdQuery &dq : g.queries) dq.n_parts = tiles;
      g.n_chunks = g.total_tiles = (uint32_t)g.queries.size() * tiles;
      continue;
    }
    if (gi == kGAll) {
      g.kpl = kpl_for(g.max_k);
      for (const TqdQuery &dq : g.queries) g.total_tiles += dq.n_parts;
      g.n_chunks = g.total_tiles;
      continue;
    }
    const int rc = gi == kGUShare   ? build_share_plan(b.s, g, ps)
                   : gi == kGAShare ? build_ashare_plan(b.s, g, ps, false, alone ? ashare_resident(b.cus) : 0u)
                   : gi == kGBShare ? build_ashare_plan(b.s, g, ps, true)
                   : gi == kGXUnion ? build_dense_plan(b.s, g, ps, (uint32_t)std::max(1, b.cus))
                                    : build_group_chunks(g, b.or_windows && gi != kGBool, ps, gi == kGBool);
    if (rc == TQ_ERR_UNSUPPORTED && (gi == kGAShare || gi == kGBShare) && ps.ap[gi == kGBShare ? 1 : 0].over_budget) {
      (gi == kGBShare ? b.co.no_bshare : b.co.no_ashare) = true;
      b.replan = true;
    }
    if (rc != TQ_OK) return rc;
  }
  for (int gi = 0; gi < kNGroups; ++gi) {
    Group &g = b.groups[gi];
    b.part_off_bytes[gi] = b.partial_bytes;
    if (kGroupTraits[gi].result_lists) {
      if (!g.queries.empty())
        b.partial_bytes += std::max<size_t>((size_t)g.list_entries, (size_t)g.queries.back().part_start + g.queries.back().n_parts) * sizeof(uint64_t);
      continue;
    }
    uint32_t parts = 0;
    for (TqdQuery &dq : g.queries) {
      dq.part_start = parts;
      parts += dq.n_parts;
    }
    b.partial_bytes += (size_t)parts * (size_t)g.kpl * 64u * sizeof(uint64_t);
  }
  Group &tree = b.groups[kGTree];
  for (size_t i = 0; i < tree.tree.size(); ++i) tree.tree[i].part_start = tree.queries[i].part_start;
  Group &all = b.groups[kGAll];
  for (size_t i = 0; i < all.all.size(); ++i) all.all[i].part_start = all.queries[i].part_start;
  Group &slop = b.groups[kGSlop];
  for (size_t i = 0; i < slop.slop.size(); ++i) slop.slop[i].part_start = slop.queries[i].part_start;
  return TQ_OK;
}

int plan_batch(Batch &b) {
  b.t0 = Clock::now();
  b.exhaustive = b.co.exhaustive;
  int rc = sync_term_records(b);
  if (rc != TQ_OK) return rc;
  look_at_queries(b);
  b.or_windows = b.s->opt.or_windows < 0 ? b.exhaustive : b.s->opt.or_windows != 0;
  if ((rc = build_flat_probe_tables(b)) != TQ_OK || (rc = build_tree_probe_tables(b)) != TQ_OK || (rc = build_all_probe_tables(b)) != TQ_OK) return rc;
  count_leaders(b);
  build_leader_norms(b);
  if ((rc = route_queries(b)) != TQ_OK) return rc;
  return plan_group_tasks(b);
}

int lay_out_stage(Batch &b) {
  if (!b.sc->ev_last) HIP_TRY(hipEventCreateWithFlags(&b.sc->ev_last, hipEventDisableTiming));
  int rc = b.sc->partials.ensure(b.partial_bytes + 256);
  if (rc == TQ_OK) rc = b.s->d_qmatches.ensure((size_t)b.n_queries * sizeof(uint32_t));
  if (rc != TQ_OK) return rc;
  const PlanScratch &ps = *b.ps;
  b.copies.reserve(8 * kNGroups + b.caches.size());
  auto put = [&](size_t align, const void *src, size_t bytes) {
    b.stage = (b.stage + align - 1) & ~(align - 1);
    if (bytes && src) b.copies.push_back({b.stage, src, bytes});
    b.stage += bytes;
    return b.stage - bytes;
  };
  for (const float *c : b.caches) put(1, c, 256 * sizeof(float));
  for (int gi = 0; gi < kNGroups; ++gi) {
    Group &g = b.groups[gi];
    if (g.queries.empty()) continue;
    if (gi == kGAShare) {
      g.o_queries = put(16, nullptr, g.queries.size() * sizeof(TqdAQuery));
      g.o_xqueries = put(16, nullptr, (size_t)b.t.n_ashare_ext * sizeof(TqdQuery));
    } else {
      g.o_queries = put(16, g.queries.data(), g.queries.size() * sizeof(TqdQuery));
    }
    g.o_tiles = put(16, g.tile_starts.data(), g.tile_starts.size() * sizeof(uint32_t));
    g.o_outidx = put(16, g.out_index.data(), g.out_index.size() * sizeof(uint32_t));
    g.o_chunks = put(16, g.chunk_recs.data(), g.chunk_recs.size() * sizeof(uint4));
    g.o_sinks = put(16, nullptr, sizeof(TqkSinks));
    if (gi == kGUShare) {
      g.o_leads = put(64, ps.leads.data(), ps.leads.size() * sizeof(TqdLead));
      g.o_tasks = put(16, ps.tasks.data(), ps.tasks.size() * sizeof(uint4));
    } else if (gi == kGAShare || gi == kGBShare) {
      const PlanScratch::ASharePlan &A = ps.ap[gi == kGBShare ? 1 : 0];
      g.o_leads = put(64, A.aleads.data(), A.aleads.size() * sizeof(TqdALead));
      g.o_tasks = put(16, A.atasks.data(), A.atasks.size() * sizeof(uint4));
      g.o_lists = put(16, A.alists.data(), gi == kGBShare ? A.alists.size() * sizeof(uint2) : 0);
    } else if (gi == kGTree) {
      g.o_leads = put(64, g.tree.data(), g.tree.size() * sizeof(TqdTreeQuery));
    } else if (gi == kGAll) {
      g.o_leads = put(64, g.all.data(), g.all.size() * sizeof(TqdAllQuery));
    } else if (gi == kGSlop) {
      g.o_leads = put(64, g.slop.data(), g.slop.size() * sizeof(TqdSlopQuery));
    } else if (gi == kGXUnion) {
      g.o_leads = put(64, ps.xrows.data(), ps.xrows.size() * sizeof(TqkDenseRow));
      g.o_tasks = put(16, ps.xqueries.data(), ps.xqueries.size() * sizeof(TqkDenseQuery));
    }
  }
  b.o_terms = put(16, b.s->h_dterms.data() + b.terms_from, (b.terms_to - b.terms_from) * sizeof(TqdTerm));
  b.t_laid = Clock::now();
  return TQ_OK;
}

int fill_stage(Batch &b) {
  if (b.s->stage_in_flight) {
    HIP_TRY(hipEventSynchronize(b.s->ev_stage_done));
    b.s->stage_in_flight = false;
  }
  b.t_waited = Clock::now();
  b.bx = (int)(b.s->batches_enqueued & 1u);
  int rc = b.s->h_stage.ensure(b.stage);
  if (rc == TQ_OK) rc = b.s->d_stage.ensure(b.stage);
  if (rc == TQ_OK) rc = b.s->d_stage_alt.ensure(b.stage);
  if (rc != TQ_OK) return rc;
  b.ds = (const uint8_t *)(b.bx ? b.s->d_stage_alt : b.s->d_stage).p;
  uint8_t *hs = (uint8_t *)b.s->h_stage.p;
  for (const Batch::Copy &c : b.copies) {
    const uint32_t parts = c.bytes >= (1u << 20) ? std::min<uint32_t>(plan_threads(), 4u) : 1u;
    parallel_slabs(parts, [&](uint32_t pi) {
      const size_t x = (c.bytes * pi / parts) & ~(size_t)63, y = pi + 1 == parts ? c.bytes : (c.bytes * (pi + 1) / parts) & ~(size_t)63;
      memcpy(hs + c.off + x, (const uint8_t *)c.src + x, y - x);
    });
  }
  {
    const Group &g = b.groups[kGAShare];
    TqdAQuery *aq = (TqdAQuery *)(hs + g.o_queries);
    TqdQuery *xq = (TqdQuery *)(hs + g.o_xqueries);
    uint32_t n_ext = 0;
    for (size_t q = 0; q < g.queries.size(); ++q) {
      const TqdQuery &dq = g.queries[q];
      TqdAQuery r{};
      r.part_start = dq.part_start;
      r.chunk_first = dq.chunk_first;
      r.k = dq.k;
      r.term1 = dq.term[1];
      r.n_terms = dq.n_terms;
      r.ext = 0xFFFFFFFFu;
      if (dq.n_terms > 2u) {
        if (n_ext == b.t.n_ashare_ext) return fail(TQ_ERR_INVALID, "shared intersections: more queries of three and more lists than were routed");
        r.ext = n_ext;
        xq[n_ext++] = dq;
      }
      aq[q] = r;
    }
  }
  for (int gi = 0; gi < kNGroups; ++gi) {
    const Group &g = b.groups[gi];
    if (g.queries.empty()) continue;
    TqkSinks sk{};
    sk.partials = (uint64_t *)((uint8_t *)b.sc->partials.p + b.part_off_bytes[gi]);
    sk.match_counter = b.s->d_match_counter;
    sk.query_matches = (uint32_t *)b.s->d_qmatches.p;
    sk.out_index = (const uint32_t *)(b.ds + g.o_outidx);
    memcpy(hs + g.o_sinks, &sk, sizeof sk);
  }
  b.t_filled = Clock::now();
  return TQ_OK;
}

int order_batch(Batch &b) {
  b.slot = (int)(b.s->batches_timed % tq_segment::kTimingRing);
  const int rc = order_after_last_batch(b.s, b.st);
  if (rc != TQ_OK) return rc;
  if (b.sc->in_flight && b.sc->last_stream != b.st) HIP_TRY(hipStreamWaitEvent(b.st, b.sc->ev_last, 0));
  if (b.s->opt.timing) HIP_TRY(hipEventRecord(b.s->ev_t0[b.slot], b.st));
  return TQ_OK;
}

void drop_leader_mats(Batch &b) {
  for (uint32_t h : b.lmat_fill) b.s->terms[h].lmat_epoch = 0;
  b.lmat_fill.clear();
}
int fill_leader_mats(Batch &b) {
  for (uint32_t h : b.lmat_fill) {
    const hipError_t e = fill_lmat(b.s, h, b.st);
    if (e != hipSuccess) {
      drop_leader_mats(b);
      return fail(TQ_ERR_HIP, "leader doc-matrix words: %s", hipGetErrorString(e));
    }
  }
  b.lmat_fill.clear();
  return TQ_OK;
}

int enqueue_copy(Batch &b) {
  if (b.s->buf_used[b.bx]) HIP_TRY(hipStreamWaitEvent(b.s->copy_stream, b.s->ev_buf_free[b.bx], 0));
  HIP_TRY(hipMemcpyAsync((void *)b.ds, b.s->h_stage.p, b.stage, hipMemcpyHostToDevice, b.s->copy_stream));
  HIP_TRY(hipEventRecord(b.s->ev_stage_done, b.s->copy_stream));
  HIP_TRY(hipEventRecord(b.s->ev_copy_done[b.bx], b.s->copy_stream));
  HIP_TRY(hipStreamWaitEvent(b.st, b.s->ev_copy_done[b.bx], 0));
  b.s->stage_in_flight = true;
  if (b.terms_to > b.terms_from) {
    HIP_TRY(hipMemcpyAsync(b.s->d_terms + b.terms_from, b.ds + b.o_terms, (b.terms_to - b.terms_from) * sizeof(TqdTerm),
                           hipMemcpyDeviceToDevice, b.st));
    b.s->d_terms_dirty = false;
    b.s->d_terms_dirty_from = ~(size_t)0;
    b.s->d_terms_synced = b.terms_to;
  }
  return TQ_OK;
}

DevBuf &list_words(tq_segment *s, int gi) {
  return gi == kGAShare ? s->d_ashare_words : gi == kGBShare ? s->d_bshare_words : s->d_share_words;
}
DevBuf &list_stage(DeviceScratch &sc, int gi) {
  return gi == kGAShare ? sc.ashare_stage : gi == kGBShare ? sc.bshare_stage : sc.share_stage;
}

int zero_batch_buffers(Batch &b) {
  TqkZeroParams zp{};
  auto zero_later = [&](void *ptr, size_t bytes) -> int {
    if (!bytes) return TQ_OK;
    if (zp.n == (uint32_t)TQK_ZERO_MAX || (bytes & 3u) || ((uintptr_t)ptr & 3u) || bytes > 0xFFFFFFFFull * 4u) {
      HIP_TRY(hipMemsetAsync(ptr, 0, bytes, b.st));
      return TQ_OK;
    }
    zp.ptr[zp.n] = (uint32_t *)ptr;
    zp.words[zp.n++] = (uint32_t)(bytes >> 2);
    return TQ_OK;
  };
  int rc = zero_later(b.s->d_match_counter, sizeof(unsigned long long));
  if (rc == TQ_OK) rc = zero_later(b.s->d_qmatches.p, (size_t)b.n_queries * sizeof(uint32_t));
  if (rc != TQ_OK) return rc;
  b.s->last_batch_queries = b.n_queries;
  b.s->last_batch_slop = !b.groups[kGSlop].queries.empty();
  b.s->slop_over_words = b.n_queries;
  if (b.s->last_batch_slop) {
    rc = b.s->d_slop_over.ensure((size_t)b.n_queries * sizeof(uint32_t));
    if (rc == TQ_OK) rc = zero_later(b.s->d_slop_over.p, (size_t)b.n_queries * sizeof(uint32_t));
    if (rc != TQ_OK) return rc;
  }
  if (b.t.n_thr_rows) {
    const size_t thr_bytes = (size_t)b.t.n_thr_rows * TQD_THR_SLOTS * sizeof(uint32_t);
    rc = b.s->d_thr.ensure(thr_bytes);
    if (rc == TQ_OK) rc = zero_later(b.s->d_thr.p, thr_bytes);
    if (rc != TQ_OK) return rc;
  }
  static const uint32_t kGridMul = std::max<uint32_t>(1u, tune_u32("TQ_US_GRID_MUL", 16));
  static const uint32_t kAGridMul = tune_u32("TQ_AS_GRID_MUL", 0);
  const uint64_t cus = (uint64_t)std::max(1, b.cus);
  for (int gi : {kGXUnion, kGUShare, kGAShare, kGBShare}) {
    const Group &g = b.groups[gi];
    const size_t n = g.queries.size();
    if (!n) continue;
    const uint32_t per_cu = gi == kGXUnion ? 0u : gi == kGUShare ? kGridMul : kAGridMul ? kAGridMul
                            : gi == kGBShare ? tqk_bshare_waves_per_cu() : tqk_ashare_waves_per_cu();
    b.grid[gi] = gi == kGXUnion ? b.ps->xgrid : (uint32_t)std::min<uint64_t>(g.n_chunks, cus * per_cu);
    const size_t stage_lists = (size_t)b.grid[gi] * (gi == kGXUnion ? n : gi == kGUShare ? TQD_US_GROUP : TQD_AS_GROUP);
    const size_t words = 2 * n + 16;
    rc = list_words(b.s, gi).ensure(words * sizeof(uint32_t));
    if (rc == TQ_OK) rc = list_stage(*b.sc, gi).ensure(stage_lists * tqk_share_capl(g.kpl) * sizeof(uint64_t));
    if (rc == TQ_OK) rc = zero_later(list_words(b.s, gi).p, words * sizeof(uint32_t));
    if (rc != TQ_OK) return rc;
  }
  return launched(tqk_launch_zero(zp, b.st), "zero");
}

template <typename P>
void common_params(P &p, const Batch &b, const Group &g) {
  p.seg = b.s->dseg;
  p.terms = b.s->d_terms;
  p.queries = (const TqdQuery *)(b.ds + g.o_queries);
  p.caches = (const float *)(b.ds + b.o_caches);
  p.sinks = (const TqkSinks *)(b.ds + g.o_sinks);
  p.thr_slots = (uint32_t *)b.s->d_thr.p;
  p.debug = b.s->opt.debug >= 0 ? (uint32_t)b.s->opt.debug : knobs().debug;
  p.bound_slack = b.co.bound_slack;
}

int launch_ashare(const Batch &b, int gi, hipStream_t gst) {
  const Group &g = b.groups[gi];
  const int ai = gi == kGBShare ? 1 : 0;
  const size_t n_a = g.queries.size();
  TqkAShareParams ap{};
  common_params(ap, b, g);
  if (gi == kGAShare) {
    ap.queries = nullptr;
    ap.aqueries = (const TqdAQuery *)(b.ds + g.o_queries);
    ap.xqueries = (const TqdQuery *)(b.ds + g.o_xqueries);
  }
  ap.leads = (const TqdALead *)(b.ds + g.o_leads);
  ap.tasks = (const uint4 *)(b.ds + g.o_tasks);
  ap.qlists = (const uint2 *)(b.ds + g.o_lists);
  ap.thr_val = (uint32_t *)list_words(b.s, gi).p;
  ap.list_count = ap.thr_val + n_a;
  ap.table_base = (const uint8_t *)b.ps->share_table_base;
  ap.stage = (uint64_t *)list_stage(*b.sc, gi).p;
  ap.lists = (uint64_t *)((uint8_t *)b.sc->partials.p + b.part_off_bytes[gi]);
  ap.n_queries = (uint32_t)n_a;
  ap.boolean = (uint32_t)ai;
  ap.rdir_lists = ai && b.ps->ap[ai].any_rdir ? 1u : 0u;
  static const uint32_t kBoundMode = tune_u32("TQ_AS_BOUND", 3);
  ap.bound_mode = kBoundMode;
  ap.n_queues = 1;
  const uint32_t bounds[3] = {0u, b.ps->ap[ai].a_inline ? g.n_chunks : b.ps->ap[ai].a_warm_tasks, g.n_chunks};
  for (int ph = 0; ph < 2; ++ph) {
    ap.task_begin = bounds[ph];
    ap.n_tasks = bounds[ph + 1];
    if (ap.n_tasks <= ap.task_begin) continue;
    ap.task_counter = ap.thr_val + 2 * n_a + 8 * ph;
    ap.grid = std::min<uint32_t>(b.grid[gi], ap.n_tasks - ap.task_begin);
    const int rc = launched(tqk_launch_ashare(ap, g.kpl, gst), "shared-intersection");
    if (rc != TQ_OK) return rc;
  }
  return TQ_OK;
}

int launch_ushare(const Batch &b, hipStream_t gst) {
  const Group &g = b.groups[kGUShare];
  const size_t n_share = g.queries.size();
  TqkShareParams sp{};
  common_params(sp, b, g);
  sp.leads = (const TqdLead *)(b.ds + g.o_leads);
  sp.tasks = (const uint4 *)(b.ds + g.o_tasks);
  sp.thr_val = (uint32_t *)b.s->d_share_words.p;
  sp.list_count = sp.thr_val + n_share;
  uint32_t *const counters = sp.thr_val + 2 * n_share;
  sp.stage = (uint64_t *)b.sc->share_stage.p;
  sp.lists = (uint64_t *)((uint8_t *)b.sc->partials.p + b.part_off_bytes[kGUShare]);
  sp.n_queries = (uint32_t)n_share;
  sp.table_base = (const uint8_t *)b.ps->share_table_base;
  static const uint32_t kPhases = tune_u32("TQ_US_PHASES", 0);
  for (uint32_t ph = 0; ph < TQD_US_MAX_TERMS; ++ph) {
    sp.task_begin = b.ps->share_phase_first[ph];
    sp.n_tasks = b.ps->share_phase_first[ph + 1];
    if (!kPhases) {
      if (ph) break;
      sp.n_tasks = g.n_chunks;
    }
    if (sp.n_tasks <= sp.task_begin) continue;
    sp.task_counter = counters + ph;
    sp.grid = std::min<uint32_t>(b.grid[kGUShare], sp.n_tasks - sp.task_begin);
    const int rc = launched(tqk_launch_share(sp, g.kpl, gst), "shared-union");
    if (rc != TQ_OK) return rc;
  }
  return TQ_OK;
}

int launch_tree(const Batch &b, hipStream_t gst) {
  const Group &g = b.groups[kGTree];
  TqkTreeParams tp{};
  tp.seg = b.s->dseg;
  tp.terms = b.s->d_terms;
  tp.queries = (const TqdTreeQuery *)(b.ds + g.o_leads);
  tp.caches = (const float *)(b.ds + b.o_caches);
  tp.sinks = (const TqkSinks *)(b.ds + g.o_sinks);
  tp.table_base = (const uint8_t *)b.s->share_table_lo;
  tp.n_queries = (uint32_t)g.queries.size();
  tp.n_words = (b.s->max_doc + 31u) / 32u;
  bool any_field = false;
  for (const TqdTreeQuery &tq : g.tree) {
    tp.any_phrase |= tq.has_phrase;
    for (uint32_t t = 0; b.s->n_field_terms && t < tq.n_terms; ++t) any_field = any_field || (tq.atom_end[t] >> 4) != 0u;
  }
  if (any_field) {
    TqkTreeFieldsParams fp{};
    fp.base = tp;
    fp.fn[0] = b.s->d_fn;
    for (uint32_t f = 1; f < TQK_MAX_FIELDS; ++f) fp.fn[f] = b.s->d_fn_field[f];
    return launched(tqk_launch_tree_fields(fp, g.kpl, gst), "nested boolean (multi-field)");
  }
  return launched(tqk_launch_tree(tp, g.kpl, gst), "nested boolean");
}

int launch_all(const Batch &b, hipStream_t gst) {
  const Group &g = b.groups[kGAll];
  TqkAllParams ap{};
  ap.seg = b.s->dseg;
  ap.terms = b.s->d_terms;
  ap.queries = (const TqdAllQuery *)(b.ds + g.o_leads);
  ap.caches = (const float *)(b.ds + b.o_caches);
  ap.sinks = (const TqkSinks *)(b.ds + g.o_sinks);
  ap.table_base = (const uint8_t *)b.s->share_table_lo;
  ap.n_queries = (uint32_t)g.queries.size();
  ap.n_words = (b.s->max_doc + 31u) / 32u;
  for (const TqdAllQuery &aq : g.all) ap.max_tiles = std::max(ap.max_tiles, aq.n_tiles);
  return launched(tqk_launch_all(ap, g.kpl, gst), "match-all");
}

int launch_slop(const Batch &b, hipStream_t gst) {
  const Group &g = b.groups[kGSlop];
  TqkPhraseSlopParams sp{};
  sp.seg = b.s->dseg;
  sp.terms = b.s->d_terms;
  sp.queries = (const TqdSlopQuery *)(b.ds + g.o_leads);
  sp.caches = (const float *)(b.ds + b.o_caches);
  sp.sinks = (const TqkSinks *)(b.ds + g.o_sinks);
  sp.table_base = (const uint8_t *)b.s->share_table_lo;
  sp.overflow = (uint32_t *)b.s->d_slop_over.p;
  sp.n_queries = (uint32_t)g.queries.size();
  sp.n_words = (b.s->max_doc + 31u) / 32u;
  for (const TqdSlopQuery &sq : g.slop) (sq.n_terms > 2u ? sp.any_carry : sp.any_pair) = 1u;
  return launched(tqk_launch_phrase_slop(sp, g.kpl, gst), "sloppy phrase");
}

int launch_xunion(const Batch &b, hipStream_t gst) {
  const PlanScratch &ps = *b.ps;
  const Group &g = b.groups[kGXUnion];
  const size_t n_dense = g.queries.size();
  TqkDenseParams dp{};
  dp.seg = b.s->dseg;
  dp.terms = b.s->d_terms;
  dp.rows = (const TqkDenseRow *)(b.ds + g.o_leads);
  dp.queries = (const TqkDenseQuery *)(b.ds + g.o_tasks);
  dp.cache = (const float *)(b.ds + b.o_caches) + (size_t)ps.xcache * 256u;
  dp.sinks = (const TqkSinks *)(b.ds + g.o_sinks);
  dp.thr_slots = (uint32_t *)b.s->d_thr.p;
  dp.thr_val = (uint32_t *)b.s->d_share_words.p;
  dp.list_count = dp.thr_val + n_dense;
  dp.task_counter = dp.thr_val + 2 * n_dense;
  dp.stage = (uint64_t *)b.sc->share_stage.p;
  dp.lists = (uint64_t *)((uint8_t *)b.sc->partials.p + b.part_off_bytes[kGXUnion]);
  dp.n_rows = (uint32_t)ps.xrows.size();
  dp.n_bitmap_rows = ps.x_bitmap_rows;
  dp.n_queries = (uint32_t)n_dense;
  dp.max_terms = ps.x_max_terms;
  dp.n_tasks = g.n_chunks;
  dp.tiles_per_task = ps.x_tiles_per_task;
  dp.list_stride = ps.x_list_stride;
  dp.grid = b.grid[kGXUnion];
  dp.debug = knobs().debug;
  return launched(tqk_launch_xunion(dp, g.kpl, gst), "doc-major union");
}

int launch_scan(const Batch &b, int gi, hipStream_t gst) {
  const Group &g = b.groups[gi];
  TqkScanParams p{};
  common_params(p, b, g);
  if (!b.s->opt.use_dense) p.seg.docmat = nullptr, p.seg.doccls = nullptr;
  p.tile_starts = (const uint32_t *)(b.ds + g.o_tiles);
  p.n_queries = (uint32_t)g.queries.size();
  p.total_tiles = g.total_tiles;
  p.chunk_recs = (const uint4 *)(b.ds + g.o_chunks);
  p.n_chunks = g.n_chunks;
  p.exhaustive = (uint32_t)b.exhaustive;
  p.use_dense = (uint32_t)b.s->opt.use_dense;
  p.all_dense = (gi == kGAndDense || (gi == kGPhrase && b.t.phrase_all_dense)) ? 1u : 0u;
  p.or_windows = gi == kGPhSweep ? 2u : ((b.or_windows && gi != kGBool) ? 1u : 0u);
  p.boolean = gi == kGBool ? 1u : 0u;
  p.small_k = g.max_k <= 16u ? 1u : 0u;
  p.max_terms = 0;
  for (const TqdQuery &dq : g.queries) p.max_terms = std::max(p.max_terms, dq.n_terms);
  const bool dpp = b.s->opt.use_dpp != 0;
  return launched(g.mode == TQ_MODE_AND  ? tqk_launch_and(p, g.kpl, dpp, gst)
                  : g.mode == TQ_MODE_OR ? tqk_launch_or(p, g.kpl, dpp, gst)
                                         : tqk_launch_phrase(p, g.kpl, dpp, gst),
                  "scan kernel");
}

int launch_groups(Batch &b) {
  const Group *groups = b.groups;
  if (b.s->opt.timing) HIP_TRY(hipEventRecord(b.s->ev_k0[b.slot], b.st));
  const bool fork = std::count_if(groups, groups + kNGroups, [](const Group &g) { return !g.queries.empty(); }) > 1;
  if (fork) {
    HIP_TRY(hipEventRecord(b.s->ev_fork, b.st));
    HIP_TRY(hipStreamWaitEvent(b.s->side_stream, b.s->ev_fork, 0));
  }
  int main_group = -1;
  for (int gi : {kGAShare, kGAndDense, kGPhSweep})
    if (main_group < 0 && !groups[gi].queries.empty()) main_group = gi;
  for (int gi = 0; main_group < 0 && gi < kNGroups; ++gi)
    if (!groups[gi].queries.empty()) main_group = gi;
  for (const int gi : {kGAnd, kGBool, kGBShare, kGUShare, kGXUnion, kGTree, kGSlop, kGAll, kGUnion, kGPhrase, kGPhSweep, kGAndDense, kGAShare}) {
    if (groups[gi].queries.empty()) continue;
    const hipStream_t gst = (fork && gi != main_group) ? b.s->side_stream : b.st;
    const int rc = gi == kGAShare || gi == kGBShare ? launch_ashare(b, gi, gst)
                   : gi == kGUShare                ? launch_ushare(b, gst)
                   : gi == kGTree                  ? launch_tree(b, gst)
                   : gi == kGAll                   ? launch_all(b, gst)
                   : gi == kGSlop                  ? launch_slop(b, gst)
                   : gi == kGXUnion                ? launch_xunion(b, gst)
                                                   : launch_scan(b, gi, gst);
    if (rc != TQ_OK) return rc;
  }
  if (fork) {
    HIP_TRY(hipEventRecord(b.s->ev_join, b.s->side_stream));
    HIP_TRY(hipStreamWaitEvent(b.st, b.s->ev_join, 0));
  }
  if (b.s->opt.timing) HIP_TRY(hipEventRecord(b.s->ev_k1[b.slot], b.st));
  return TQ_OK;
}

int launch_merges(const Batch &b) {
  for (int gi = 0; gi < kNGroups; ++gi) {
    const Group &g = b.groups[gi];
    if (g.queries.empty()) continue;
    TqkMergeParams m{};
    m.queries = (const TqdQuery *)(b.ds + g.o_queries);
    m.partials = (const uint64_t *)((const uint8_t *)b.sc->partials.p + b.part_off_bytes[gi]);
    m.out_index = (const uint32_t *)(b.ds + g.o_outidx);
    m.out_scores = b.out_scores;
    m.out_docs = b.out_docs;
    m.out_counts = b.out_counts;
    m.out_segment_ords = b.out_segment_ords;
    m.segment_ord = b.segment_ord;
    m.n_queries = (uint32_t)g.queries.size();
    m.out_stride = b.out_stride;
    if (!kGroupTraits[gi].result_lists) {
      uint32_t max_parts = 0;
      for (const TqdQuery &dq : g.queries) max_parts = std::max(max_parts, dq.n_parts);
      if (max_parts >= TQK_MERGE_PRE_MIN && m.n_queries <= 4096u)
        m.pre_slices = std::min<uint32_t>(32u, std::max<uint32_t>(2u, (uint32_t)std::sqrt((double)max_parts)));
    }
    const int rc = launched(kGroupTraits[gi].result_lists
                                ? tqk_launch_merge_lists(m, (const uint32_t *)list_words(b.s, gi).p + g.queries.size(), g.kpl, gi == kGAShare, b.st)
                                : tqk_launch_merge(m, g.kpl, b.st),
                            "merge kernel");
    if (rc != TQ_OK) return rc;
  }
  if (b.s->last_batch_slop && b.co.h_slop_over)
    HIP_TRY(hipMemcpyAsync(b.co.h_slop_over, b.s->d_slop_over.p, (size_t)b.n_queries * sizeof(uint32_t), hipMemcpyDeviceToHost, b.st));
  return TQ_OK;
}

int finish_batch(const Batch &b) {
  DeviceScratch &sc = *b.sc;
  if (b.s->opt.timing) {
    HIP_TRY(hipEventRecord(b.s->ev_t1[b.slot], b.st));
    ++b.s->batches_timed;
  }
  HIP_TRY(hipEventRecord(b.s->ev_batch_done, b.st));
  HIP_TRY(hipEventRecord(sc.ev_last, b.st));
  sc.last_stream = b.st;
  sc.in_flight = true;
  HIP_TRY(hipEventRecord(b.s->ev_buf_free[b.bx], b.st));
  b.s->buf_used[b.bx] = true;
  ++b.s->batches_enqueued;
  b.s->last_stream = b.st;
  b.s->batch_in_flight = true;
  uint32_t kernel_mask = 0, tiles_total = 0, chunks_total = 0;
  if (b.s->opt.record_query_kernels) b.s->last_query_kernel.assign(b.n_queries, 0u);
  for (int gi = 0; gi < kNGroups; ++gi) {
    const Group &g = b.groups[gi];
    if (g.queries.empty()) continue;
    const uint32_t bit = group_kernel_bit(gi, b.or_windows);
    kernel_mask |= bit;
    tiles_total += g.total_tiles;
    chunks_total += g.n_chunks;
    if (b.s->opt.record_query_kernels)
      for (uint32_t qi : g.out_index) b.s->last_query_kernel[qi] = bit;
  }
  static const bool trace = getenv("TQ_TRACE") != nullptr;
  if (trace) {
    const auto t_enqueued = Clock::now();
    auto us = [](auto x, auto y) { return (long)std::chrono::duration_cast<std::chrono::microseconds>(y - x).count(); };
    for (int gi = 0; gi < kNGroups; ++gi)
      if (!b.groups[gi].queries.empty())
        fprintf(stderr, "[tq] group %d: %zu queries, %u tasks\n", gi, b.groups[gi].queries.size(), b.groups[gi].n_chunks);
    fprintf(stderr, "[tq] plan %ld us (pre-pass %ld us, queries %ld us, chunks %ld us), wait for the staging buffer %ld us, stage fill %ld us, enqueue %ld us, stage bytes %zu\n",
            us(b.t0, b.t_laid), us(b.t0, b.t_route), us(b.t_route, b.t_routed), us(b.t_routed, b.t_laid), us(b.t_laid, b.t_waited),
            us(b.t_waited, b.t_filled), us(b.t_filled, t_enqueued), b.stage);
  }
  b.s->stats.algorithmic_bytes = b.t.algo_bytes;
  b.s->stats.tiles = tiles_total;
  b.s->stats.chunks = chunks_total;
  b.s->stats.matches = 0;
  b.s->stats.kernel_ms = 0;
  b.s->stats.total_ms = 0;
  b.s->stats.host_plan_ms = 0;
  b.s->stats.kernel_mask = kernel_mask;
  b.s->stats.unique_bytes = b.unique_bytes;
  b.s->stats_pending = true;
  b.s->stats_match_bytes = 1;
  b.s->stats_sorted = false;
  return TQ_OK;
}

struct DrainOnError {
  tq_segment *s;
  hipStream_t st;
  bool armed = true;
  ~DrainOnError() {
    if (!armed) return;
    if (s->copy_stream) (void)hipStreamSynchronize(s->copy_stream);
    if (s->side_stream) (void)hipStreamSynchronize(s->side_stream);
    (void)hipStreamSynchronize(st);
  }
};

struct AllStrip {
  std::vector<tq_query> eff;
  std::deque<AllView> views;
  std::deque<std::array<uint8_t, TQ_MAX_TERMS>> set_occurs;
  std::vector<uint8_t> set_q;
  std::deque<TreeView> field_phrases;
  std::deque<SlopView> slop_views;
  std::vector<uint32_t> slop_q;
  uint32_t n_all_based = 0, n_set = 0;
};
int strip_all_clauses(const tq_segment *s, const tq_query *queries, uint32_t n_queries, AllStrip &st) {
  const bool sets = s->n_set_slots != 0;
  const bool fields = s->n_field_terms != 0;
  for (uint32_t qi = 0; qi < n_queries; ++qi) {
    if (queries[qi].slop) {
      st.slop_views.emplace_back();
      const int vrc = slop_view(s, queries[qi], qi, "tq_search_batch", st.slop_views.back(), true);
      if (vrc != TQ_OK) return vrc;
      if (st.eff.empty()) st.eff.assign(queries, queries + n_queries);
      st.eff[qi] = st.slop_views.back().v.q;
      if (st.slop_q.empty()) st.slop_q.assign(n_queries, 0);
      st.slop_q[qi] = queries[qi].slop;
      continue;
    }
    bool names_set = false;
    if (sets) {
      const int src = check_set_query(s, queries[qi], qi, "tq_search_batch", &names_set);
      if (src != TQ_OK) return src;
    }
    bool names_field = false;
    if (fields && query_names_field(s, queries[qi])) {
      const int frc = check_field_query(s, queries[qi], qi, "tq_search_batch");
      if (frc != TQ_OK) return frc;
      names_field = true;
      if (queries[qi].mode == TQ_MODE_PHRASE) {
        const tq_query &pq = queries[qi];
        if (pq.n_terms < 2 || !pq.phrase_offsets || !pq.weights) return fail(TQ_ERR_INVALID, "query %u: a phrase needs >= 2 terms, offsets and a weight", qi);
        if (st.eff.empty()) st.eff.assign(queries, queries + n_queries);
        st.field_phrases.emplace_back();
        docset_tree_view(pq, st.field_phrases.back(), true);
        st.eff[qi] = st.field_phrases.back().q;
        if (st.set_q.empty()) st.set_q.assign(n_queries, 0);
        st.set_q[qi] = 1;
        ++st.n_set;
        continue;
      }
    }
    bool all_based = false;
    if (query_has_all(queries[qi])) {
      AllForm f;
      const char *why = "";
      const int rc = all_query_form(queries[qi], f, &why);
      if (rc != TQ_OK) return fail(rc, "query %u: %s", qi, why);
      if (f.boost_mixed)
        return fail(TQ_ERR_UNSUPPORTED, "query %u has a boosted match-all clause beside another scoring clause or a second match-all clause: its scores stay on the CPU", qi);
      all_based = f.kind == TQ_ALL_BASED;
      if (all_based) {
        ++st.n_all_based;
      } else {
        if (st.eff.empty()) st.eff.assign(queries, queries + n_queries);
        st.views.emplace_back();
        all_strip_view(queries[qi], f, st.views.back());
        st.eff[qi] = st.views.back().q;
      }
    }
    if (!names_set && !names_field) continue;
    const tq_query &q = st.eff.empty() ? queries[qi] : st.eff[qi];
    if (all_based) {
      for (uint32_t i = 0; i < q.n_terms; ++i) {
        const bool must_not = q.mode == TQ_MODE_BOOL && q.occurs && q.occurs[i] == TQ_MUST_NOT;
        if (is_term_set(s, q.terms[i]) && !must_not)
          return fail(TQ_ERR_UNSUPPORTED, "tq_search_batch: query %u: a term set as a Should clause beside a match-all clause stays on the CPU (its counts and doc sets are taken)", qi);
        if (names_field && term_field_of(s, q.terms[i]) && !must_not)
          return fail(TQ_ERR_UNSUPPORTED, "tq_search_batch: query %u: a Should term of field %u (the scoring terms of a query whose match-all clauses make every doc a candidate are its Should terms) stays on the CPU (its counts and doc sets are taken)", qi, term_field_of(s, q.terms[i]));
      }
      continue;
    }
    if (!(names_set && query_names_set(s, q)) && !(names_field && query_names_field(s, q))) continue;
    if (st.set_q.empty()) st.set_q.assign(n_queries, 0);
    st.set_q[qi] = 1;
    ++st.n_set;
    if (q.mode == TQ_MODE_BOOL) continue;
    if (st.eff.empty()) st.eff.assign(queries, queries + n_queries);
    st.set_occurs.emplace_back();
    st.set_occurs.back().fill(q.mode == TQ_MODE_AND ? (uint8_t)TQ_MUST : (uint8_t)TQ_SHOULD);
    tq_query &v = st.eff[qi];
    v.mode = TQ_MODE_BOOL;
    v.occurs = st.set_occurs.back().data();
    v.clause_of = v.nested_occurs = v.clause_min_should = v.atom_of = nullptr;
    v.min_should_match = 0;
  }
  return TQ_OK;
}

size_t host_rows_layout(uint32_t n_queries, uint32_t out_stride, size_t &o_docs, size_t &o_counts) {
  const size_t n = (size_t)n_queries * out_stride;
  o_docs = (n * sizeof(float) + 255) & ~(size_t)255;
  o_counts = (o_docs + n * sizeof(uint32_t) + 255) & ~(size_t)255;
  return o_counts + (size_t)n_queries * sizeof(uint32_t);
}

}

int search_batch_impl(tq_segment *s, const tq_query *queries, uint32_t n_queries,
                      uint32_t out_stride, float *d_out_scores, uint32_t *d_out_docs,
                      uint32_t *d_out_counts, void *hip_stream, const CallOpts &co, uint32_t *d_out_segment_ords,
                      uint32_t segment_ord) {
  if (!s || (!queries && n_queries) || !d_out_scores || !d_out_docs || !d_out_counts)
    return fail(TQ_ERR_INVALID, "tq_search_batch: null argument");
  if (n_queries == 0) return TQ_OK;
  AllStrip strip;
  int rc = strip_all_clauses(s, queries, n_queries, strip);
  if (rc != TQ_OK) return rc;
  if (!strip.eff.empty()) queries = strip.eff.data();
  Batch b{s, queries, n_queries, out_stride, d_out_scores, d_out_docs, d_out_counts, hip_stream, co, d_out_segment_ords, segment_ord};
  b.n_all_queries = strip.n_all_based;
  b.set_q = strip.n_set ? strip.set_q.data() : nullptr;
  b.slop_q = strip.slop_q.empty() ? nullptr : strip.slop_q.data();
  rc = plan_batch(b);
  while (rc != TQ_OK && b.replan) {
    drop_leader_mats(b);
    b = Batch{s, queries, n_queries, out_stride, d_out_scores, d_out_docs, d_out_counts, hip_stream, b.co, d_out_segment_ords, segment_ord};
    b.n_all_queries = strip.n_all_based;
    b.set_q = strip.n_set ? strip.set_q.data() : nullptr;
    b.slop_q = strip.slop_q.empty() ? nullptr : strip.slop_q.data();
    rc = plan_batch(b);
  }
  struct DropMats {
    Batch &b;
    ~DropMats() { drop_leader_mats(b); }
  } drop_mats{b};
  if (rc != TQ_OK) return rc;
  b.sc = s->dscratch;
  std::unique_lock<std::mutex> scratch_lock(b.sc->m);
  if ((rc = lay_out_stage(b)) != TQ_OK || (rc = fill_stage(b)) != TQ_OK || (rc = order_batch(b)) != TQ_OK || (rc = fill_leader_mats(b)) != TQ_OK) return rc;
  DrainOnError drain_on_error{s, b.st};
  if ((rc = enqueue_copy(b)) != TQ_OK || (rc = zero_batch_buffers(b)) != TQ_OK || (rc = launch_groups(b)) != TQ_OK ||
      (rc = launch_merges(b)) != TQ_OK || (rc = finish_batch(b)) != TQ_OK)
    return rc;
  drain_on_error.armed = false;
  s->host_ms_sum += std::chrono::duration<double, std::milli>((Clock::now() - b.t0) - (b.t_waited - b.t_laid)).count();
  ++s->host_ms_n;
  return TQ_OK;
}

int resolve_opts(const tq_segment *s, const tq_search_opts *o, CallOpts &co) {
  co.exhaustive = __atomic_load_n(&s->opt.exhaustive, __ATOMIC_RELAXED) != 0;
  uint32_t ppm = (uint32_t)__atomic_load_n(&s->opt.bound_slack_ppm, __ATOMIC_RELAXED);
  if (o) {
    if (o->exhaustive == 0 || o->exhaustive == 1)
      co.exhaustive = o->exhaustive != 0;
    else if (o->exhaustive != -1)
      return fail(TQ_ERR_INVALID, "tq_search_opts.exhaustive must be -1, 0 or 1");
    if (o->bound_slack_ppm != TQ_OPT_DEFAULT) ppm = o->bound_slack_ppm;
    if (ppm > 1000000000u) return fail(TQ_ERR_INVALID, "bound_slack_ppm above 1e9");
  }
  co.bound_slack = 1.0f + (float)ppm * 1e-6f;
  return TQ_OK;
}

int search_batch_host(tq_segment *s, const tq_query *queries, uint32_t n_queries,
                      uint32_t out_stride, float *out_scores, uint32_t *out_docs,
                      uint32_t *out_counts, const CallOpts &co) {
  if (!s || !out_scores || !out_docs || !out_counts)
    return fail(TQ_ERR_INVALID, "tq_search_batch: null argument");
  if (n_queries == 0) return TQ_OK;
  HIP_TRY(hipSetDevice(s->device));
  const size_t n = (size_t)n_queries * out_stride;
  size_t o_docs, o_counts;
  const size_t o_over = (host_rows_layout(n_queries, out_stride, o_docs, o_counts) + 255) & ~(size_t)255;
  int rc = s->h_out.ensure(o_over + (size_t)n_queries * sizeof(uint32_t));
  if (rc != TQ_OK) return rc;
  uint8_t *h = (uint8_t *)s->h_out.p;
  CallOpts co_over = co;
  co_over.h_slop_over = (uint32_t *)(h + o_over);
  rc = search_batch_impl(s, queries, n_queries, out_stride, (float *)h, (uint32_t *)(h + o_docs),
                         (uint32_t *)(h + o_counts), nullptr, co_over);
  if (rc != TQ_OK) return rc;
  HIP_TRY(hipStreamSynchronize(s->stream));
  memcpy(out_scores, h, n * sizeof(float));
  memcpy(out_docs, h + o_docs, n * sizeof(uint32_t));
  memcpy(out_counts, h + o_counts, (size_t)n_queries * sizeof(uint32_t));
  if (co.defer_slop_verdict) {
    if (s->last_batch_slop) s->slop_over_host.assign((const uint32_t *)(h + o_over), (const uint32_t *)(h + o_over) + n_queries);
    return TQ_OK;
  }
  return s->last_batch_slop ? slop_overflow_verdict("tq_search_batch", (const uint32_t *)(h + o_over), n_queries) : TQ_OK;
}
int search_batch_host_begin(tq_segment *s, const tq_query *queries, uint32_t n_queries, uint32_t out_stride,
                            const CallOpts &co, HostBatchSlot &slot) {
  if (!s || !n_queries) return fail(TQ_ERR_INVALID, "tq_submit: empty batch");
  HIP_TRY(hipSetDevice(s->device));
  slot.n = n_queries;
  slot.stride = out_stride;
  slot.o_slop_over = (host_rows_layout(n_queries, out_stride, slot.o_docs, slot.o_counts) + 255) & ~(size_t)255;
  int rc = slot.out.ensure(slot.o_slop_over + (size_t)n_queries * sizeof(uint32_t));
  if (rc != TQ_OK) return rc;
  if (!slot.done) HIP_TRY(hipEventCreateWithFlags(&slot.done, hipEventDisableTiming));
  if (!slot.done_blocking) HIP_TRY(hipEventCreateWithFlags(&slot.done_blocking, hipEventDisableTiming | hipEventBlockingSync));
  uint8_t *h = (uint8_t *)slot.out.p;
  CallOpts co_over = co;
  co_over.h_slop_over = (uint32_t *)(h + slot.o_slop_over);
  rc = search_batch_impl(s, queries, n_queries, out_stride, (float *)h, (uint32_t *)(h + slot.o_docs),
                         (uint32_t *)(h + slot.o_counts), nullptr, co_over);
  if (rc != TQ_OK) return rc;
  slot.any_slop = s->last_batch_slop;
  static const uint32_t kBlockMin = tune_u32("TQ_SUBMIT_BLOCK_MIN", 128);
  slot.blocking = n_queries >= kBlockMin;
  HIP_TRY(hipEventRecord(slot.blocking ? slot.done_blocking : slot.done, s->stream));
  return TQ_OK;
}
int search_batch_host_end(tq_segment *s, HostBatchSlot &slot) {
  (void)s;
  HIP_TRY(hipEventSynchronize(slot.blocking ? slot.done_blocking : slot.done));
  return TQ_OK;
}
}

extern "C" {

int tq_search_batch_device(tq_segment *s, const tq_query *queries, uint32_t n_queries,
                           uint32_t out_stride, float *d_out_scores, uint32_t *d_out_docs,
                           uint32_t *d_out_counts, void *hip_stream) {
  return tq_search_batch_device_opts(s, queries, n_queries, out_stride, d_out_scores, d_out_docs,
                                     d_out_counts, nullptr, hip_stream);
}

int tq_search_batch_device_opts(tq_segment *s, const tq_query *queries, uint32_t n_queries,
                                uint32_t out_stride, float *d_out_scores, uint32_t *d_out_docs,
                                uint32_t *d_out_counts, const tq_search_opts *opts,
                                void *hip_stream) {
  if (!s) return fail(TQ_ERR_INVALID, "tq_search_batch: null segment");
  try {
    TQ_SEGMENT_LOCK(s);
    CallOpts co;
    const int rc = resolve_opts(s, opts, co);
    if (rc != TQ_OK) return rc;
    return search_batch_impl(s, queries, n_queries, out_stride, d_out_scores, d_out_docs,
                             d_out_counts, hip_stream, co);
  } catch (const std::exception &e) {
    return fail(TQ_ERR_HIP, "tq_search_batch_device: %s", e.what());
  } catch (...) {
    return fail(TQ_ERR_HIP, "tq_search_batch_device: unknown exception");
  }
}

int tq_search_batch_device_rows(tq_segment *s, const tq_query *queries, uint32_t n_queries,
                                uint32_t out_stride, float *d_out_scores, uint32_t *d_out_segment_ords,
                                uint32_t *d_out_docs, uint32_t *d_out_counts, uint32_t segment_ord,
                                const tq_search_opts *opts, void *hip_stream) {
  if (!s) return fail(TQ_ERR_INVALID, "tq_search_batch: null segment");
  if (!d_out_segment_ords) return fail(TQ_ERR_INVALID, "tq_search_batch_device_rows: null argument");
  try {
    TQ_SEGMENT_LOCK(s);
    CallOpts co;
    const int rc = resolve_opts(s, opts, co);
    if (rc != TQ_OK) return rc;
    return search_batch_impl(s, queries, n_queries, out_stride, d_out_scores, d_out_docs,
                             d_out_counts, hip_stream, co, d_out_segment_ords, segment_ord);
  } catch (const std::exception &e) {
    return fail(TQ_ERR_HIP, "tq_search_batch_device_rows: %s", e.what());
  } catch (...) {
    return fail(TQ_ERR_HIP, "tq_search_batch_device_rows: unknown exception");
  }
}

int tq_search_batch(tq_segment *s, const tq_query *queries, uint32_t n_queries,
                    uint32_t out_stride, float *out_scores, uint32_t *out_docs,
                    uint32_t *out_counts) {
  return tq_search_batch_opts(s, queries, n_queries, out_stride, out_scores, out_docs, out_counts,
                              nullptr);
}

int tq_search_batch_opts(tq_segment *s, const tq_query *queries, uint32_t n_queries,
                         uint32_t out_stride, float *out_scores, uint32_t *out_docs,
                         uint32_t *out_counts, const tq_search_opts *opts) {
  if (!s) return fail(TQ_ERR_INVALID, "tq_search_batch: null segment");
  try {
    TQ_SEGMENT_LOCK(s);
    CallOpts co;
    const int rc = resolve_opts(s, opts, co);
    if (rc != TQ_OK) return rc;
    return search_batch_host(s, queries, n_queries, out_stride, out_scores, out_docs, out_counts, co);
  } catch (const std::exception &e) {
    return fail(TQ_ERR_HIP, "tq_search_batch: %s", e.what());
  } catch (...) {
    return fail(TQ_ERR_HIP, "tq_search_batch: unknown exception");
  }
}

// ... 2 lines not shown
```

Baseline: 12.39 million queries/s.

## Zero batch buffers on copy stream with double-buffered sinks, fewer events

```diff
diff --git a/tantivy_amd/csrc/tq_api.cpp b/tantivy_amd/csrc/tq_api.cpp
--- a/tantivy_amd/csrc/tq_api.cpp
+++ b/tantivy_amd/csrc/tq_api.cpp
@@ -95,7 +95,6 @@
   if (rc == TQ_OK && fieldnorm) rc = up(&s->d_fn, fieldnorm, max_doc);
   if (rc == TQ_OK) {
     hipError_t e = hipStreamCreateWithFlags(&s->stream, hipStreamNonBlocking);
-    if (e == hipSuccess) e = hipEventCreateWithFlags(&s->ev_stage_done, hipEventDisableTiming);
     if (e == hipSuccess) e = hipEventCreateWithFlags(&s->ev_fork, hipEventDisableTiming);
     if (e == hipSuccess) e = hipEventCreateWithFlags(&s->ev_join, hipEventDisableTiming);
     if (e == hipSuccess) e = hipEventCreateWithFlags(&s->ev_batch_done, hipEventDisableTiming);
@@ -112,6 +111,7 @@
       if (e == hipSuccess) e = hipEventCreate(&s->ev_k1[i]);
     }
     if (e == hipSuccess) e = hipMalloc((void **)&s->d_match_counter, 6u * sizeof(unsigned long long));
+    if (e == hipSuccess) e = hipMalloc((void **)&s->d_match_counter_alt, 6u * sizeof(unsigned long long));
     if (e == hipSuccess) e = hipMalloc((void **)&s->d_tp_info, 2 * sizeof(TqpInfo));
     if (e != hipSuccess) rc = fail(TQ_ERR_HIP, "segment setup: %s", hipGetErrorString(e));
   }
@@ -233,7 +233,15 @@
   if (!s) return;
   (void)hipSetDevice(s->device);
   if (s->stream) (void)hipStreamSynchronize(s->stream);
-  if (s->batch_in_flight && s->ev_batch_done) (void)hipEventSynchronize(s->ev_batch_done);
+  if (s->batch_in_flight && s->ev_batch_end) (void)hipEventSynchronize(s->ev_batch_end);
+  if (s->dscratch) {
+    std::lock_guard<std::mutex> lk(s->dscratch->m);
+    if (s->dscratch->ev_last_owner == s) {
+      s->dscratch->ev_last = nullptr;
+      s->dscratch->ev_last_owner = nullptr;
+      s->dscratch->in_flight = false;
+    }
+  }
   for (void *slab : s->term_slabs) (void)hipFree(slab);
   dense_arena_free(s);
   for (void *ptr : s->dense_extra) (void)hipFree(ptr);
@@ -249,6 +257,7 @@
   if (s->d_tp_info) (void)hipFree(s->d_tp_info);
   if (s->d_local_cache) (void)hipFree(s->d_local_cache);
   if (s->d_match_counter) (void)hipFree(s->d_match_counter);
+  if (s->d_match_counter_alt) (void)hipFree(s->d_match_counter_alt);
   s->d_stage.release();
   s->d_misc.release();
   for (int i = 0; i < 2; ++i) {
@@ -265,6 +274,8 @@
   s->d_share_words.release();
   s->d_ashare_words.release();
   s->d_bshare_words.release();
+  for (DevBuf *alt : {&s->d_thr_alt, &s->d_qmatches_alt, &s->d_share_words_alt, &s->d_ashare_words_alt, &s->d_bshare_words_alt, &s->d_slop_over_alt})
+    alt->release();
   s->d_count_queries.release();
   s->d_count_out.release();
   s->d_count_bits.release();
@@ -295,7 +306,7 @@
   s->h_out.release();
   if (s->side_stream) (void)hipStreamSynchronize(s->side_stream);
   if (s->copy_stream) (void)hipStreamSynchronize(s->copy_stream);
-  for (hipEvent_t ev : {s->ev_stage_done, s->ev_fork, s->ev_join, s->ev_batch_done, s->ev_copy_done[0],
+  for (hipEvent_t ev : {s->ev_fork, s->ev_join, s->ev_batch_done, s->ev_copy_done[0],
                         s->ev_copy_done[1], s->ev_buf_free[0], s->ev_buf_free[1]})
     if (ev) (void)hipEventDestroy(ev);
   if (s->side_stream) (void)hipStreamDestroy(s->side_stream);
@@ -313,13 +324,13 @@
 namespace tqi {
 int order_after_last_batch(tq_segment *s, hipStream_t st) {
   if (s->batch_in_flight && s->last_stream != st)
-    HIP_TRY(hipStreamWaitEvent(st, s->ev_batch_done, 0));
+    HIP_TRY(hipStreamWaitEvent(st, s->ev_batch_end, 0));
   return TQ_OK;
 }
 int wait_segment_idle(tq_segment *s) {
   HIP_TRY(hipStreamSynchronize(s->stream));
   if (s->batch_in_flight) {
-    HIP_TRY(hipEventSynchronize(s->ev_batch_done));
+    HIP_TRY(hipEventSynchronize(s->ev_batch_end));
     s->batch_in_flight = false;
   }
   return TQ_OK;
@@ -367,7 +378,7 @@
     const int wrc = wait_segment_idle(s);
     if (wrc != TQ_OK) return wrc;
   }
-  HIP_TRY(hipMemcpy(out, s->d_qmatches.p, (size_t)n * sizeof(uint32_t), hipMemcpyDeviceToHost));
+  HIP_TRY(hipMemcpy(out, s->set_qmatches(s->last_set).p, (size_t)n * sizeof(uint32_t), hipMemcpyDeviceToHost));
   return TQ_OK;
 }
 
@@ -476,7 +487,7 @@
       }
       s->stats_sorted = false;
     } else {
-      HIP_TRY(hipMemcpy(&m, s->d_match_counter, sizeof m, hipMemcpyDeviceToHost));
+      HIP_TRY(hipMemcpy(&m, s->set_match_counter(s->last_set), sizeof m, hipMemcpyDeviceToHost));
       s->stats.matches = m;
       s->stats.algorithmic_bytes += m * s->stats_match_bytes;
     }
@@ -489,7 +500,7 @@
       for (uint64_t b = first; b < s->batches_timed; ++b) {
         const int i = (int)(b % tq_segment::kTimingRing);
         float km = 0, tm = 0;
-        if (hipEventElapsedTime(&km, s->ev_k0[i], s->ev_k1[i]) == hipSuccess &&
+        if (hipEventElapsedTime(&km, s->k0_is_t0[i] ? s->ev_t0[i] : s->ev_k0[i], s->ev_k1[i]) == hipSuccess &&
             hipEventElapsedTime(&tm, s->ev_t0[i], s->ev_t1[i]) == hipSuccess) {
           k_sum += km;
           t_sum += tm;
@@ -536,6 +547,7 @@
   r.docmat_bytes = s->bytes_docmat;
   r.posdir_bytes = s->bytes_posdir;
   r.scratch_bytes = s->d_stage.cap + s->d_stage_alt.cap + s->d_misc.cap + s->d_thr.cap + s->d_qmatches.cap + s->d_share_words.cap +
+                    s->d_thr_alt.cap + s->d_qmatches_alt.cap + s->d_share_words_alt.cap + s->d_ashare_words_alt.cap + s->d_bshare_words_alt.cap + s->d_slop_over_alt.cap +
                     s->d_ashare_words.cap + s->d_bshare_words.cap + s->d_count_queries.cap + s->d_count_out.cap +
                     s->d_count_bits.cap + s->d_count_wgs.cap + s->d_set_work.cap + s->docset_scratch_bytes();
   {
diff --git a/tantivy_amd/csrc/tq_count.cpp b/tantivy_amd/csrc/tq_count.cpp
--- a/tantivy_amd/csrc/tq_count.cpp
+++ b/tantivy_amd/csrc/tq_count.cpp
@@ -154,6 +154,7 @@
   std::vector<tq_query> eff;
   std::vector<uint8_t> done;
   const tq_query *const given = queries;
+  s->last_set = 0;
   s->last_batch_slop = false;
   for (uint32_t qi = 0; qi < n_queries; ++qi) {
     if (!query_has_all(given[qi])) continue;
diff --git a/tantivy_amd/csrc/tq_docset.cpp b/tantivy_amd/csrc/tq_docset.cpp
--- a/tantivy_amd/csrc/tq_docset.cpp
+++ b/tantivy_amd/csrc/tq_docset.cpp
@@ -550,7 +550,10 @@
 int run_device(const Batch &b) {
   tq_segment *const s = b.s;
   const DocsetCall &call = b.call;
-  if (b.timed) HIP_TRY(hipEventRecord(s->ev_k0[b.ring], b.st));
+  if (b.timed) {
+    HIP_TRY(hipEventRecord(s->ev_k0[b.ring], b.st));
+    s->k0_is_t0[b.ring] = false;
+  }
   int rc = sweep(b, DS_SCATTER | DS_COUNT | DS_WRITE, call.out_docs, call.out_scores, call.out_cap);
   if (rc == TQ_OK && call.consumer == Consumer::kAgg) rc = agg_finish(s, *call.agg, b.n_queries, b.st);
   if (rc != TQ_OK) return rc;
@@ -569,6 +572,7 @@
   s->stats_agg_terms_sub = call.agg && call.agg->terms_sub;
   s->stats_agg_terms_hist_row = call.agg && call.agg->terms_hist ? call.agg->plan.n_buckets + 1u : 0u;
   HIP_TRY(hipEventRecord(s->ev_batch_done, b.st));
+  s->ev_batch_end = s->ev_batch_done;
   s->last_stream = b.st;
   s->batch_in_flight = true;
   return TQ_OK;
@@ -621,6 +625,7 @@
   b.dqs.resize(n_queries);
   b.sqs.resize(call.scored ? n_queries : 0u);
   s->last_batch_slop = false;
+  s->last_set = 0;
   s->slop_over_words = b.n_over_words();
   int rc = check_and_express(b);
   if (rc == TQ_OK) rc = plan_trees(b);
diff --git a/tantivy_amd/csrc/tq_internal.hpp b/tantivy_amd/csrc/tq_internal.hpp
--- a/tantivy_amd/csrc/tq_internal.hpp
+++ b/tantivy_amd/csrc/tq_internal.hpp
@@ -194,6 +194,7 @@
   std::mutex m;
   DevBuf partials, share_stage, ashare_stage, bshare_stage;
   hipEvent_t ev_last = nullptr;
+  const void *ev_last_owner = nullptr;
   hipStream_t last_stream = nullptr;
   bool in_flight = false;
 };
@@ -210,7 +211,6 @@
   ~tq_ctx() {
     for (auto &kv : scratch) {
       (void)hipSetDevice(kv.first);
-      if (kv.second->ev_last) (void)hipEventDestroy(kv.second->ev_last);
       kv.second->partials.release();
       kv.second->share_stage.release();
       kv.second->ashare_stage.release();
@@ -317,21 +317,31 @@
   bool last_batch_slop = false;
   uint32_t slop_over_words = 0;
   std::vector<uint32_t> slop_over_host;
+  DevBuf d_thr_alt, d_qmatches_alt, d_share_words_alt, d_ashare_words_alt, d_bshare_words_alt, d_slop_over_alt;
+  unsigned long long *d_match_counter_alt = nullptr;
+  int last_set = 0;
+  DevBuf &set_thr(int x) { return x ? d_thr_alt : d_thr; }
+  DevBuf &set_qmatches(int x) { return x ? d_qmatches_alt : d_qmatches; }
+  DevBuf &set_slop_over(int x) { return x ? d_slop_over_alt : d_slop_over; }
+  unsigned long long *set_match_counter(int x) { return x ? d_match_counter_alt : d_match_counter; }
   std::vector<uint32_t> last_query_kernel;
   PinnedBuf h_stage, h_out;
   static constexpr int kTimingRing = 16;
-  hipEvent_t ev_stage_done = nullptr, ev_fork = nullptr, ev_join = nullptr;
-  hipEvent_t ev_batch_done = nullptr;
+  hipEvent_t ev_fork = nullptr, ev_join = nullptr;
+  hipEvent_t ev_stage_done = nullptr;
+  hipEvent_t ev_batch_done = nullptr, ev_batch_end = nullptr;
   hipStream_t last_stream = nullptr;
   bool batch_in_flight = false;
   hipStream_t side_stream = nullptr;
   hipStream_t copy_stream = nullptr;
   DevBuf d_stage_alt;
-  hipEvent_t ev_copy_done[2] = {nullptr, nullptr}, ev_buf_free[2] = {nullptr, nullptr};
+  hipEvent_t ev_copy_done[2] = {nullptr, nullptr}, ev_buf_free[2] = {nullptr, nullptr}, ev_buf_end[2] = {nullptr, nullptr};
+  int cus = 0;
   bool buf_used[2] = {false, false};
   uint64_t batches_enqueued = 0;
   hipEvent_t ev_t0[kTimingRing] = {}, ev_t1[kTimingRing] = {}, ev_k0[kTimingRing] = {},
              ev_k1[kTimingRing] = {};
+  bool k0_is_t0[kTimingRing] = {};
   uint64_t batches_timed = 0, batches_reported = 0;
   bool stage_in_flight = false;
   double host_ms_sum = 0;
diff --git a/tantivy_amd/csrc/tq_phrase_slop.cpp b/tantivy_amd/csrc/tq_phrase_slop.cpp
--- a/tantivy_amd/csrc/tq_phrase_slop.cpp
+++ b/tantivy_amd/csrc/tq_phrase_slop.cpp
@@ -82,7 +82,7 @@
 int slop_overflow_readback(tq_segment *s, const char *fn) {
   if (!s->last_batch_slop) return TQ_OK;
   std::vector<uint32_t> over(s->slop_over_words);
-  HIP_TRY(hipMemcpy(over.data(), s->d_slop_over.p, over.size() * sizeof(uint32_t), hipMemcpyDeviceToHost));
+  HIP_TRY(hipMemcpy(over.data(), s->set_slop_over(s->last_set).p, over.size() * sizeof(uint32_t), hipMemcpyDeviceToHost));
   return slop_overflow_verdict(fn, over.data(), (uint32_t)over.size());
 }
 
@@ -103,6 +103,6 @@
     const int wrc = wait_segment_idle(s);
     if (wrc != TQ_OK) return wrc;
   }
-  HIP_TRY(hipMemcpy(out, s->d_slop_over.p, (size_t)n * sizeof(uint32_t), hipMemcpyDeviceToHost));
+  HIP_TRY(hipMemcpy(out, s->set_slop_over(s->last_set).p, (size_t)n * sizeof(uint32_t), hipMemcpyDeviceToHost));
   return TQ_OK;
 }
diff --git a/tantivy_amd/csrc/tq_search.cpp b/tantivy_amd/csrc/tq_search.cpp
--- a/tantivy_amd/csrc/tq_search.cpp
+++ b/tantivy_amd/csrc/tq_search.cpp
@@ -49,6 +49,9 @@
   std::vector<Copy> copies;
   size_t stage = 0, o_caches = 0, o_terms = 0;
   int bx = 0;
+  int set = 0;
+  bool zero_on_copy = false;
+  bool one_t0 = false;
   const uint8_t *ds = nullptr;
   DeviceScratch *sc = nullptr;
   int slot = 0;
@@ -823,7 +826,8 @@
 
 int plan_group_tasks(Batch &b) {
   PlanScratch &ps = *b.ps;
-  (void)hipDeviceGetAttribute(&b.cus, hipDeviceAttributeMultiprocessorCount, b.s->device);
+  if (b.s->cus <= 0 && hipDeviceGetAttribute(&b.s->cus, hipDeviceAttributeMultiprocessorCount, b.s->device) != hipSuccess) b.s->cus = 0;
+  if (b.s->cus > 0) b.cus = b.s->cus;
   const bool alone = std::count_if(b.groups, b.groups + kNGroups, [](const Group &g) { return !g.queries.empty(); }) == 1;
   for (int gi = 0; gi < kNGroups; ++gi) {
     Group &g = b.groups[gi];
@@ -891,9 +895,12 @@
 }
 
 int lay_out_stage(Batch &b) {
-  if (!b.sc->ev_last) HIP_TRY(hipEventCreateWithFlags(&b.sc->ev_last, hipEventDisableTiming));
+  static const bool kZeroOnCopy = tune_u32("TQ_ZERO_ON_COPY", 1) != 0;
+  b.bx = (int)(b.s->batches_enqueued & 1u);
+  b.zero_on_copy = kZeroOnCopy;
+  b.set = b.zero_on_copy ? b.bx : 0;
   int rc = b.sc->partials.ensure(b.partial_bytes + 256);
-  if (rc == TQ_OK) rc = b.s->d_qmatches.ensure((size_t)b.n_queries * sizeof(uint32_t));
+  if (rc == TQ_OK) rc = b.s->set_qmatches(b.set).ensure((size_t)b.n_queries * sizeof(uint32_t));
   if (rc != TQ_OK) return rc;
   const PlanScratch &ps = *b.ps;
   b.copies.reserve(8 * kNGroups + b.caches.size());
@@ -947,7 +954,6 @@
     b.s->stage_in_flight = false;
   }
   b.t_waited = Clock::now();
-  b.bx = (int)(b.s->batches_enqueued & 1u);
   int rc = b.s->h_stage.ensure(b.stage);
   if (rc == TQ_OK) rc = b.s->d_stage.ensure(b.stage);
   if (rc == TQ_OK) rc = b.s->d_stage_alt.ensure(b.stage);
@@ -988,8 +994,8 @@
     if (g.queries.empty()) continue;
     TqkSinks sk{};
     sk.partials = (uint64_t *)((uint8_t *)b.sc->partials.p + b.part_off_bytes[gi]);
-    sk.match_counter = b.s->d_match_counter;
-    sk.query_matches = (uint32_t *)b.s->d_qmatches.p;
+    sk.match_counter = b.s->set_match_counter(b.set);
+    sk.query_matches = (uint32_t *)b.s->set_qmatches(b.set).p;
     sk.out_index = (const uint32_t *)(b.ds + g.o_outidx);
     memcpy(hs + g.o_sinks, &sk, sizeof sk);
   }
@@ -1002,7 +1008,8 @@
   const int rc = order_after_last_batch(b.s, b.st);
   if (rc != TQ_OK) return rc;
   if (b.sc->in_flight && b.sc->last_stream != b.st) HIP_TRY(hipStreamWaitEvent(b.st, b.sc->ev_last, 0));
-  if (b.s->opt.timing) HIP_TRY(hipEventRecord(b.s->ev_t0[b.slot], b.st));
+  b.one_t0 = b.zero_on_copy && b.lmat_fill.empty() && b.terms_to == b.terms_from;
+  if (b.s->opt.timing && !b.one_t0) HIP_TRY(hipEventRecord(b.s->ev_t0[b.slot], b.st));
   return TQ_OK;
 }
 
@@ -1022,11 +1029,17 @@
   return TQ_OK;
 }
 
+int zero_batch_buffers(Batch &b, hipStream_t zst);
 int enqueue_copy(Batch &b) {
-  if (b.s->buf_used[b.bx]) HIP_TRY(hipStreamWaitEvent(b.s->copy_stream, b.s->ev_buf_free[b.bx], 0));
+  if (b.s->buf_used[b.bx]) HIP_TRY(hipStreamWaitEvent(b.s->copy_stream, b.s->ev_buf_end[b.bx], 0));
   HIP_TRY(hipMemcpyAsync((void *)b.ds, b.s->h_stage.p, b.stage, hipMemcpyHostToDevice, b.s->copy_stream));
-  HIP_TRY(hipEventRecord(b.s->ev_stage_done, b.s->copy_stream));
+  if (b.zero_on_copy) {
+    if (b.s->batch_in_flight && b.s->ev_batch_end == b.s->ev_batch_done) HIP_TRY(hipStreamWaitEvent(b.s->copy_stream, b.s->ev_batch_end, 0));
+    const int zrc = zero_batch_buffers(b, b.s->copy_stream);
+    if (zrc != TQ_OK) return zrc;
+  }
   HIP_TRY(hipEventRecord(b.s->ev_copy_done[b.bx], b.s->copy_stream));
+  b.s->ev_stage_done = b.s->ev_copy_done[b.bx];
   HIP_TRY(hipStreamWaitEvent(b.st, b.s->ev_copy_done[b.bx], 0));
   b.s->stage_in_flight = true;
   if (b.terms_to > b.terms_from) {
@@ -1039,40 +1052,42 @@
   return TQ_OK;
 }
 
-DevBuf &list_words(tq_segment *s, int gi) {
+DevBuf &list_words(tq_segment *s, int gi, int set) {
+  if (set) return gi == kGAShare ? s->d_ashare_words_alt : gi == kGBShare ? s->d_bshare_words_alt : s->d_share_words_alt;
   return gi == kGAShare ? s->d_ashare_words : gi == kGBShare ? s->d_bshare_words : s->d_share_words;
 }
 DevBuf &list_stage(DeviceScratch &sc, int gi) {
   return gi == kGAShare ? sc.ashare_stage : gi == kGBShare ? sc.bshare_stage : sc.share_stage;
 }
 
-int zero_batch_buffers(Batch &b) {
+int zero_batch_buffers(Batch &b, hipStream_t zst) {
   TqkZeroParams zp{};
   auto zero_later = [&](void *ptr, size_t bytes) -> int {
     if (!bytes) return TQ_OK;
     if (zp.n == (uint32_t)TQK_ZERO_MAX || (bytes & 3u) || ((uintptr_t)ptr & 3u) || bytes > 0xFFFFFFFFull * 4u) {
-      HIP_TRY(hipMemsetAsync(ptr, 0, bytes, b.st));
+      HIP_TRY(hipMemsetAsync(ptr, 0, bytes, zst));
       return TQ_OK;
     }
     zp.ptr[zp.n] = (uint32_t *)ptr;
     zp.words[zp.n++] = (uint32_t)(bytes >> 2);
     return TQ_OK;
   };
-  int rc = zero_later(b.s->d_match_counter, sizeof(unsigned long long));
-  if (rc == TQ_OK) rc = zero_later(b.s->d_qmatches.p, (size_t)b.n_queries * sizeof(uint32_t));
+  int rc = zero_later(b.s->set_match_counter(b.set), sizeof(unsigned long long));
+  if (rc == TQ_OK) rc = zero_later(b.s->set_qmatches(b.set).p, (size_t)b.n_queries * sizeof(uint32_t));
   if (rc != TQ_OK) return rc;
+  b.s->last_set = b.set;
   b.s->last_batch_queries = b.n_queries;
   b.s->last_batch_slop = !b.groups[kGSlop].queries.empty();
   b.s->slop_over_words = b.n_queries;
   if (b.s->last_batch_slop) {
-    rc = b.s->d_slop_over.ensure((size_t)b.n_queries * sizeof(uint32_t));
-    if (rc == TQ_OK) rc = zero_later(b.s->d_slop_over.p, (size_t)b.n_queries * sizeof(uint32_t));
+    rc = b.s->set_slop_over(b.set).ensure((size_t)b.n_queries * sizeof(uint32_t));
+    if (rc == TQ_OK) rc = zero_later(b.s->set_slop_over(b.set).p, (size_t)b.n_queries * sizeof(uint32_t));
     if (rc != TQ_OK) return rc;
   }
   if (b.t.n_thr_rows) {
     const size_t thr_bytes = (size_t)b.t.n_thr_rows * TQD_THR_SLOTS * sizeof(uint32_t);
-    rc = b.s->d_thr.ensure(thr_bytes);
-    if (rc == TQ_OK) rc = zero_later(b.s->d_thr.p, thr_bytes);
+    rc = b.s->set_thr(b.set).ensure(thr_bytes);
+    if (rc == TQ_OK) rc = zero_later(b.s->set_thr(b.set).p, thr_bytes);
     if (rc != TQ_OK) return rc;
   }
   static const uint32_t kGridMul = std::max<uint32_t>(1u, tune_u32("TQ_US_GRID_MUL", 16));
@@ -1087,12 +1102,12 @@
     b.grid[gi] = gi == kGXUnion ? b.ps->xgrid : (uint32_t)std::min<uint64_t>(g.n_chunks, cus * per_cu);
     const size_t stage_lists = (size_t)b.grid[gi] * (gi == kGXUnion ? n : gi == kGUShare ? TQD_US_GROUP : TQD_AS_GROUP);
     const size_t words = 2 * n + 16;
-    rc = list_words(b.s, gi).ensure(words * sizeof(uint32_t));
+    rc = list_words(b.s, gi, b.set).ensure(words * sizeof(uint32_t));
     if (rc == TQ_OK) rc = list_stage(*b.sc, gi).ensure(stage_lists * tqk_share_capl(g.kpl) * sizeof(uint64_t));
-    if (rc == TQ_OK) rc = zero_later(list_words(b.s, gi).p, words * sizeof(uint32_t));
+    if (rc == TQ_OK) rc = zero_later(list_words(b.s, gi, b.set).p, words * sizeof(uint32_t));
     if (rc != TQ_OK) return rc;
   }
-  return launched(tqk_launch_zero(zp, b.st), "zero");
+  return launched(tqk_launch_zero(zp, zst), "zero");
 }
 
 template <typename P>
@@ -1102,7 +1117,7 @@
   p.queries = (const TqdQuery *)(b.ds + g.o_queries);
   p.caches = (const float *)(b.ds + b.o_caches);
   p.sinks = (const TqkSinks *)(b.ds + g.o_sinks);
-  p.thr_slots = (uint32_t *)b.s->d_thr.p;
+  p.thr_slots = (uint32_t *)b.s->set_thr(b.set).p;
   p.debug = b.s->opt.debug >= 0 ? (uint32_t)b.s->opt.debug : knobs().debug;
   p.bound_slack = b.co.bound_slack;
 }
@@ -1121,7 +1136,7 @@
   ap.leads = (const TqdALead *)(b.ds + g.o_leads);
   ap.tasks = (const uint4 *)(b.ds + g.o_tasks);
   ap.qlists = (const uint2 *)(b.ds + g.o_lists);
-  ap.thr_val = (uint32_t *)list_words(b.s, gi).p;
+  ap.thr_val = (uint32_t *)list_words(b.s, gi, b.set).p;
   ap.list_count = ap.thr_val + n_a;
   ap.table_base = (const uint8_t *)b.ps->share_table_base;
   ap.stage = (uint64_t *)list_stage(*b.sc, gi).p;
@@ -1152,7 +1167,7 @@
   common_params(sp, b, g);
   sp.leads = (const TqdLead *)(b.ds + g.o_leads);
   sp.tasks = (const uint4 *)(b.ds + g.o_tasks);
-  sp.thr_val = (uint32_t *)b.s->d_share_words.p;
+  sp.thr_val = (uint32_t *)list_words(b.s, kGUShare, b.set).p;
   sp.list_count = sp.thr_val + n_share;
   uint32_t *const counters = sp.thr_val + 2 * n_share;
   sp.stage = (uint64_t *)b.sc->share_stage.p;
@@ -1226,7 +1241,7 @@
   sp.caches = (const float *)(b.ds + b.o_caches);
   sp.sinks = (const TqkSinks *)(b.ds + g.o_sinks);
   sp.table_base = (const uint8_t *)b.s->share_table_lo;
-  sp.overflow = (uint32_t *)b.s->d_slop_over.p;
+  sp.overflow = (uint32_t *)b.s->set_slop_over(b.set).p;
   sp.n_queries = (uint32_t)g.queries.size();
   sp.n_words = (b.s->max_doc + 31u) / 32u;
   for (const TqdSlopQuery &sq : g.slop) (sq.n_terms > 2u ? sp.any_carry : sp.any_pair) = 1u;
@@ -1244,8 +1259,8 @@
   dp.queries = (const TqkDenseQuery *)(b.ds + g.o_tasks);
   dp.cache = (const float *)(b.ds + b.o_caches) + (size_t)ps.xcache * 256u;
   dp.sinks = (const TqkSinks *)(b.ds + g.o_sinks);
-  dp.thr_slots = (uint32_t *)b.s->d_thr.p;
-  dp.thr_val = (uint32_t *)b.s->d_share_words.p;
+  dp.thr_slots = (uint32_t *)b.s->set_thr(b.set).p;
+  dp.thr_val = (uint32_t *)list_words(b.s, kGXUnion, b.set).p;
   dp.list_count = dp.thr_val + n_dense;
   dp.task_counter = dp.thr_val + 2 * n_dense;
   dp.stage = (uint64_t *)b.sc->share_stage.p;
@@ -1289,7 +1304,10 @@
 
 int launch_groups(Batch &b) {
   const Group *groups = b.groups;
-  if (b.s->opt.timing) HIP_TRY(hipEventRecord(b.s->ev_k0[b.slot], b.st));
+  if (b.s->opt.timing) {
+    HIP_TRY(hipEventRecord(b.one_t0 ? b.s->ev_t0[b.slot] : b.s->ev_k0[b.slot], b.st));
+    b.s->k0_is_t0[b.slot] = b.one_t0;
+  }
   const bool fork = std::count_if(groups, groups + kNGroups, [](const Group &g) { return !g.queries.empty(); }) > 1;
   if (fork) {
     HIP_TRY(hipEventRecord(b.s->ev_fork, b.st));
@@ -1342,27 +1360,29 @@
         m.pre_slices = std::min<uint32_t>(32u, std::max<uint32_t>(2u, (uint32_t)std::sqrt((double)max_parts)));
     }
     const int rc = launched(kGroupTraits[gi].result_lists
-                                ? tqk_launch_merge_lists(m, (const uint32_t *)list_words(b.s, gi).p + g.queries.size(), g.kpl, gi == kGAShare, b.st)
+                                ? tqk_launch_merge_lists(m, (const uint32_t *)list_words(b.s, gi, b.set).p + g.queries.size(), g.kpl, gi == kGAShare, b.st)
                                 : tqk_launch_merge(m, g.kpl, b.st),
                             "merge kernel");
     if (rc != TQ_OK) return rc;
   }
   if (b.s->last_batch_slop && b.co.h_slop_over)
-    HIP_TRY(hipMemcpyAsync(b.co.h_slop_over, b.s->d_slop_over.p, (size_t)b.n_queries * sizeof(uint32_t), hipMemcpyDeviceToHost, b.st));
+    HIP_TRY(hipMemcpyAsync(b.co.h_slop_over, b.s->set_slop_over(b.set).p, (size_t)b.n_queries * sizeof(uint32_t), hipMemcpyDeviceToHost, b.st));
   return TQ_OK;
 }
 
 int finish_batch(const Batch &b) {
   DeviceScratch &sc = *b.sc;
-  if (b.s->opt.timing) {
-    HIP_TRY(hipEventRecord(b.s->ev_t1[b.slot], b.st));
-    ++b.s->batches_timed;
-  }
-  HIP_TRY(hipEventRecord(b.s->ev_batch_done, b.st));
-  HIP_TRY(hipEventRecord(sc.ev_last, b.st));
+  static const bool kOneEnd = tune_u32("TQ_ONE_END_EVENT", 1) != 0;
+  const hipEvent_t ev_end = b.s->opt.timing && kOneEnd ? b.s->ev_t1[b.slot] : b.s->ev_buf_free[b.bx];
+  if (b.s->opt.timing && !kOneEnd) HIP_TRY(hipEventRecord(b.s->ev_t1[b.slot], b.st));
+  HIP_TRY(hipEventRecord(ev_end, b.st));
+  if (b.s->opt.timing) ++b.s->batches_timed;
+  b.s->ev_batch_end = ev_end;
+  sc.ev_last = ev_end;
+  sc.ev_last_owner = b.s;
   sc.last_stream = b.st;
   sc.in_flight = true;
-  HIP_TRY(hipEventRecord(b.s->ev_buf_free[b.bx], b.st));
+  b.s->ev_buf_end[b.bx] = ev_end;
   b.s->buf_used[b.bx] = true;
   ++b.s->batches_enqueued;
   b.s->last_stream = b.st;
@@ -1553,7 +1573,7 @@
   std::unique_lock<std::mutex> scratch_lock(b.sc->m);
   if ((rc = lay_out_stage(b)) != TQ_OK || (rc = fill_stage(b)) != TQ_OK || (rc = order_batch(b)) != TQ_OK || (rc = fill_leader_mats(b)) != TQ_OK) return rc;
   DrainOnError drain_on_error{s, b.st};
-  if ((rc = enqueue_copy(b)) != TQ_OK || (rc = zero_batch_buffers(b)) != TQ_OK || (rc = launch_groups(b)) != TQ_OK ||
+  if ((rc = enqueue_copy(b)) != TQ_OK || (!b.zero_on_copy && (rc = zero_batch_buffers(b, b.st)) != TQ_OK) || (rc = launch_groups(b)) != TQ_OK ||
       (rc = launch_merges(b)) != TQ_OK || (rc = finish_batch(b)) != TQ_OK)
     return rc;
   drain_on_error.armed = false;
```

Result: no change. 12.53 million queries/s, median of 6 (+1.1%).
